# ucas-vg/PointTinyBenchmark

Hardware: AMD Instinct MI355X
Metric: img/s (640x640) CPR R50-FPN fwd+loss (higher is better)
Workload: dtype fp32

## Files before the change

### include/cpr_hip.h

```cpp
#ifndef CPR_HIP_H
#define CPR_HIP_H
#ifdef __cplusplus
extern "C" {
#endif

#define CPR_ERR_ARG (-1001)
#define CPR_ERR_UNSUPPORTED (-1002)

int cpr_version(void);

#define CPR_CONV_RELU 1
#define CPR_CONV_OUT_BF16 2
#define CPR_CONV_RES_MASK 4
#define CPR_CONV_COLSUM 8
int cpr_conv2d_fwd(const float* in, const float* wgt, float* out, const float* scale, const float* bias,
                   const float* residual, const float* in_a, const float* in_b, float* gn_part, int N, int H, int W,
                   int Cin, int Cout, int KH, int KW, int stride, int pad, int Kpad, int flags, int in_relu,
                   int* variant_out, void* stream);
int cpr_conv2d_fwd_dil(const float* in, const float* wgt, float* out, const float* scale, const float* bias,
                       const float* residual, const float* in_a, const float* in_b, float* gn_part, int N, int H, int W,
                       int Cin, int Cout, int KH, int KW, int stride, int pad, int dil, int Kpad, int flags, int in_relu,
                       int* variant_out, void* stream);

int cpr_conv2d_dual_fwd(const float* in, const float* wgt, const float* in2, const float* wgt2, float* out,
                        const float* scale, const float* bias, const float* scale2, const float* bias2, int N, int H, int W,
                        int Cin, int Cout, int KH, int KW, int stride, int pad, int Kpad, int H2, int W2, int Cin2,
                        int stride2, int Kpad2, int flags, int* variant_out, void* stream);

int cpr_conv1x1_stream_fwd(const float* in, const float* wgt, float* out, const float* scale, const float* bias,
                           const float* residual, long long M, int Cin, int Cout, int flags, void* stream);

int cpr_conv_wgrad_bf16_workspace_s(int N, int H, int W, int Cin, int Cout, int k, int stride, int dy_bf16, int x_bf16);
int cpr_conv_wgrad_bf16_s(const void* dy, int dy_bf16, const void* x, int x_bf16, float* grad, void* ws, int N, int H, int W, int Cin,
                          int Cout, int k, int stride, int accumulate, void* stream);

#define CPR_WINO_IN_B8 1
#define CPR_WINO_OUT_B8 2
int cpr_wino_pack_weights(const float* wgt, float* u, int Cin, int Cout, int Kpad, void* stream);
int cpr_conv3x3_wino_fwd(const float* in, const float* u, float* out, const float* scale, const float* bias,
                         const float* in_a, const float* in_b, float* gn_part, int N, int H, int W, int Cin, int Cout,
                         int flags, int in_relu, int layout, void* stream);
int cpr_wino32_pack_weights(const float* wgt, float* u, int Cin, int Cout, int Kpad, void* stream);
int cpr_conv3x3_wino32_slots(int H, int W);
int cpr_conv3x3_wino32_fwd(const float* in, const float* u, float* out, const float* scale, const float* bias,
                           const float* in_a, const float* in_b, float* gn_part, int N, int H, int W, int Cin, int Cout,
                           int flags, int in_relu, int layout, void* stream);
int cpr_gn_apply_b8(const float* x, const float* a, const float* b, float* y, int N, int H, int W, int C, int relu,
                    void* stream);

int cpr_conv2d_fwd_bf16(const void* in, const void* wgt, const void* wgt_frag, void* out, const float* scale, const float* bias,
                        const void* residual, float* gn_part, int N, int H, int W, int Cin, int Cout, int KH, int KW,
                        int stride, int pad, int Kpad, int relu, int out_fp32, int* variant_out, void* stream);
int cpr_conv2d_bf16_mask_slots(int N, int H, int W, int Cin, int Cout, int KH, int KW, int stride, int pad, int out_fp32);
int cpr_conv2d_dgrad_bf16_fused(const void* in, const void* wgt, const void* wgt_frag, float* out32, void* out16, const float* add32,
                                const void* mask, float* part, int N, int H, int W, int Cin, int Cout, int KH, int KW, int stride,
                                int pad, int Kpad, int* variant_out, void* stream);
int cpr_stem7x7s2_bf16(const float* in, const void* wgt, const float* scale, const float* bias, void* out, int N, int H, int W,
                       int relu, int layout, void* stream);
int cpr_stem7x7s2_pool_bf16(const float* in, const void* wgt, const float* scale, const float* bias, void* out, int N, int H,
                            int W, int layout, void* stream);
int cpr_maxpool3x3s2_bf16(const void* in, void* out, int N, int H, int W, int C, void* stream);
int cpr_gn_stats_bf16(const void* x, float* part, int N, int HW, int C, int P, void* stream);
int cpr_gn_apply_bf16(const void* x, const float* a, const float* b, const void* up, void* y, int N, int H, int W,
                      int C, int UH, int UW, int relu, void* stream);

int cpr_nchw_to_nhwc4(const float* in, float* out, int N, int C, int H, int W, void* stream);
int cpr_nhwc_to_nchw(const float* in, float* out, int N, int C, int H, int W, void* stream);
int cpr_stem7x7s2_pool_f32(const float* in, const float* wgt, const float* scale, const float* bias, float* out, int N, int H,
                           int W, int layout, void* stream);
int cpr_maxpool3x3s2(const float* in, float* out, int N, int H, int W, int C, void* stream);
int cpr_stem_deep_fwd(const float* in, const float* w1, const float* s1, const float* b1, const float* w2, const float* s2,
                      const float* b2, const float* w3, const float* s3, const float* b3, float* mid1, float* mid2, void* out, int N,
                      int H, int W, int layout, int out_bf16, void* stream);
int cpr_stem3x3s2_fwd(const float* in, const float* w, const float* scale, const float* bias, float* out, int N, int H, int W,
                      int layout, void* stream);
int cpr_stem3x3s2_wgrad_workspace(int N, int H, int W);
int cpr_stem3x3s2_wgrad(const float* dy, const float* in, float* gw, float* ws, int N, int H, int W, int layout, void* stream);
int cpr_avgpool_fwd(const void* in, void* out, int N, int H, int W, int C, int s, int bf16, void* stream);
int cpr_avgpool_bwd(const void* g, const void* add, void* dx, int N, int H, int W, int C, int s, int bf16, void* stream);
int cpr_maxpool3x3s2_rec(const float* in, float* out, unsigned char* arg, int N, int H, int W, int C, void* stream);
int cpr_maxpool3x3s2_bf16_rec(const void* in, void* out, unsigned char* arg, int N, int H, int W, int C, void* stream);
int cpr_stem7x7s2_pool_f32_rec(const float* in, const float* wgt, const float* scale, const float* bias, float* out,
                               unsigned char* arg, int N, int H, int W, int layout, void* stream);
int cpr_stem7x7s2_pool_bf16_rec(const float* in, const void* wgt, const float* scale, const float* bias, void* out,
                                unsigned char* arg, int N, int H, int W, int layout, void* stream);
int cpr_stem_pool_bwd_blocks(long long M);
int cpr_stem_pool_bwd(const float* dp, const unsigned char* arg, float* dy, float* part, int N, int OH, int OW, void* stream);
int cpr_stem_wgrad_f32_workspace(int N, int H, int W);
int cpr_stem_wgrad_f32(const float* dy, const float* in, float* gw, float* ws, int N, int H, int W, int layout, void* stream);

int cpr_gn_stats(const float* x, float* part, int N, int HW, int C, int P, void* stream);
int cpr_gn_finalize(const float* part, const float* gamma, const float* beta, float* a_out, float* b_out,
                    float* mean_out, float* rstd_out, int N, int P, int C, int G, int HW, float eps, void* stream);
int cpr_gn_apply(const float* x, const float* a, const float* b, const float* up, float* y, int N, int H, int W,
                 int C, int UH, int UW, int relu, void* stream);

int cpr_box_centers(const float* boxes, float* centers, int n, void* stream);

#define CPR_PROB_SIGMOID 0
#define CPR_PROB_SOFTMAX 1
#define CPR_PROB_NORMED_SIGMOID 2
#define CPR_PROB_IDENTITY 3

int cpr_logit_project(const float* x, const float* w, const float* bias, const float* in_a, const float* in_b,
                      float* out, int N, int HW, int Cin, int J, int in_relu, void* stream);

int cpr_neg_mask_loss(const float* logit, int J, const float* centers, const int* labels, const int* gt_start,
                      const int* pad_hw, unsigned char* mask, double* partial, int N, int H, int W, int C,
                      float stride, float d2_thr, float eps, int class_wise, int prob_type, float norm_p,
                      int mask_classes, int* n_partial, void* stream);

int cpr_bag_sample(const float* map, int J, const float* centers, const int* gt_img, const int* pad_hw,
                   const float* offsets, float* pts, unsigned char* valid, float* out, int G, int K, int H, int W,
                   float stride, int align_corners, const float* pad_value, void* stream);

int cpr_grid_bag(const float* map, int J, const float* points, const int* gt_img, int R, int Kmax, float radius_px,
                 const float* pad_value, float* pts, unsigned char* valid, int* ws_cell, int* count, float* out, int G,
                 int H, int W, float stride, int align_corners, void* stream);

int cpr_mil_loss(const float* logits, int J, int ins_off, const unsigned char* valid, const int* labels,
                 const float* gt_weight, float* bag_ws, const double* neg_partial, int n_partial, int num_bags,
                 int bag_stride, int bag_off, int bag_len, int ctr_off, int ctr_stride, int ctr_count, int ctr_mod,
                 int C, float eps, int prob_type, float norm_p, int binary_ins, int allpos, float w_mil, float w_gt,
                 float w_neg, int neg_from_gt, float* out5, void* stream);

int cpr_refine(const float* logits, int J, const float* pts, const unsigned char* valid, const float* centers, int Rv,
               int ctr_stride, const int* labels, const int* gt_img, const int* gt_start, const int* img_hw,
               const unsigned char* not_refine_in, float* refine_pts, float* scores, unsigned char* not_refine,
               unsigned char* chosen, int G, int Kt, int Kv, int C, int prob_type, float norm_p, float gt_alpha,
               float merge_th, float refine_th, int use_nearest, int use_classify, int score_max, void* stream);

int cpr_point_assign(const float* points, const float* gt_bboxes, int n, int k, float scale, int pos_num,
                     long long* gt_inds, float* ws_best, int* ws_lvl, void* stream);

int cpr_hungarian_cost(const float* pred, int pred_stride, const float* logits, int C, const float* gt,
                       const int* labels, float* costT, int M, int G, float w_cls, float alpha, float gamma,
                       float eps, float w_dis, float fx, float fy, int p_norm, void* stream);
int cpr_match_cost(const float* pred, int pdim, const float* logits, int C, const float* gt, const int* labels, float* costT,
                   int M, int G, const float* terms, int ncls, int nreg, void* stream);

int cpr_lsa_topk(const float* costT, const int* m_of, const int* g_of, const long long* cost_off,
                 const long long* col_off, const long long* row_off, int num_problems, int topk, long long* gt_inds,
                 double* ws_v, double* ws_spc, int* ws_path, int* ws_row4col, unsigned char* ws_sc,
                 unsigned char* ws_active, int* ws_cols, int* ws_remaining, int* ws_pos, double* ws_u,
                 int* ws_col4row, unsigned char* ws_sr, int* status, int max_cols, int max_rows, void* stream);

int cpr_topk_desc(const float* scores, int n, int k, float* out_vals, long long* out_idx, void* stream);

int cpr_nms_candidates(const float* boxes, int box_stride, const float* scores, const float* factors, int n, int C,
                       float score_thr, float* cand_boxes, float* cand_scores, int* cand_labels, long long* cand_inds,
                       int* count, void* stream);
int cpr_nms_workspace(int n);
int cpr_nms(const float* boxes, const float* scores, const int* labels, int n, float iou_thr, long long* keep_idx,
            int* num_keep, int* ws_order, float* ws_boxes, unsigned long long* ws_mask, void* stream);
int cpr_topk_desc_batched(const float* scores, int B, int n, int k, float* out_vals, long long* out_idx, void* stream);
int cpr_nms_candidates_batched(const float* boxes, int box_stride, const float* scores, const float* factors, int B, int n,
                               int C, float score_thr, float* cand_boxes, float* cand_scores, int* cand_labels,
                               long long* cand_inds, int* count, void* stream);
int cpr_nms_batched(const float* boxes, const float* scores, const int* labels, const int* n_dev, int B, int cap,
                    float iou_thr, long long* keep_idx, int* num_keep, int* ws_order, float* ws_boxes,
                    unsigned long long* ws_mask, long long ws_stride, void* stream);

int cpr_p2p_decode(const float* reg, const float* point_anchor, float* pred, float* anchor, int N, int H, int W, int k,
                   float stride, float gamma, void* stream);
int cpr_tap_sum3x3(const float* R, const float* bias, float* out, int N, int H, int W, int J, void* stream);
int cpr_rowmax_sigmoid(const float* logits, float* out, long long M, int C, void* stream);
int cpr_sigmoid(const float* x, float* y, long long n, void* stream);
int cpr_p2p_loss(const float* logits, const float* pred, const long long* gt_inds, const float* gt_pts,
                 const int* gt_labels, const int* gt_start, double* ws_partial, float* out, int B, int M, int C,
                 float alpha, float gamma, float beta, float pos_w, float neg_w, float reg_norm, float w_cls,
                 float w_reg, int cls_mode, int reg_mode, void* stream);

int cpr_conv2d_wgrad_workspace(int N, int OH, int OW, int Cin, int Cout, int KH, int KW);
int cpr_conv2d_wgrad(const float* dy, const float* x, const float* in_a, const float* in_b, float* grad_w, float* ws,
                     int N, int H, int W, int Cin, int Cout, int KH, int KW, int stride, int pad, int in_relu,
                     int accumulate, void* stream);
int cpr_conv2d_wgrad_dil(const float* dy, const float* x, float* grad_w, float* ws, int N, int H, int W, int Cin, int Cout, int KH,
                         int KW, int stride, int pad, int dil, int accumulate, void* stream);
int cpr_conv3x3_wino_wgrad_workspace(int N, int H, int W, int Cin, int Cout);
int cpr_conv3x3_wino_wgrad(const float* dy, const float* x, const float* in_a, const float* in_b, float* grad_w, float* ws,
                           int N, int H, int W, int Cin, int Cout, int in_relu, int accumulate, void* stream);
int cpr_gn_bwd(const float* x, const float* dz, const float* a, const float* b, const float* mean, const float* rstd,
               const float* gamma, float* dx, float* dgamma, float* dbeta, float* ws_part, float* ws_k, int N, int HW,
               int C, int G, int P, int relu, int accumulate, void* stream);
int cpr_gn_bwd_bf16(const void* x_bf16, const float* dz, const float* a, const float* b, const float* mean, const float* rstd,
                    const float* gamma, float* dx, void* dx_bf16, float* dgamma, float* dbeta, float* ws_part, float* ws_k, int N,
                    int HW, int C, int G, int P, int relu, int accumulate, void* stream);
int cpr_gn_bwd_bf16_dz16(const void* x_bf16, const void* dz_bf16, const float* a, const float* b, const float* mean, const float* rstd,
                         const float* gamma, float* dx, void* dx_bf16, float* dgamma, float* dbeta, float* ws_part, float* ws_k,
                         int N, int HW, int C, int G, int P, int relu, int accumulate, void* stream);
int cpr_upsample_add_bwd(const float* dfine, float* dcoarse, int N, int H, int W, int UH, int UW, int C, int accumulate,
                         void* stream);
int cpr_relu_bwd_colsum_ws(long long M, int C);
int cpr_relu_bwd_colsum(const float* dy, const float* add, const void* y, int y_bf16, float* g_out, void* g16_out, float* colsum,
                        float* ws_part, long long M, int C, int accumulate, void* stream);
int cpr_part_colsum(const float* part, float* out, float* ws, int tiles, int C, void* stream);
int cpr_bn_fold_bwd(float* Gw, const float* weight, const float* scale, const float* mean, const float* inv_sigma,
                    const float* colsum_g, float* dgamma, float* dbeta, int Cout, int K, void* stream);
int cpr_bn_fold_bwd_part(float* Gw, const float* weight, const float* scale, const float* mean, const float* inv_sigma, const float* part,
                         int tiles, float* dgamma, float* dbeta, int Cout, int K, void* stream);
int cpr_axpby(float* y, const float* x, float alpha, float beta, long long n, void* stream);
int cpr_phase_scatter_add(const float* src, float* dst, int N, int Hs, int Ws, int C, int H, int W, int py, int px,
                          int sh, int sw, int s, void* stream);
int cpr_zero_insert(const float* dy, float* out, int N, int OH, int OW, int C, int H, int W, int s, void* stream);
int cpr_pack_weights_grouped(const float* w, const float* scale, float* out, int C, int cg, int transpose, void* stream);
int cpr_pack_weights_grouped_multi(const void* jobs_dev, int n, int total_blocks, void* stream);
int cpr_conv_group_fwd(const float* x, const float* wp, float* out, const float* scale, const float* bias, int N, int H, int W, int C,
                       int cg, int stride, int flags, void* stream);
int cpr_conv_group_wgrad_workspace(int N, int OH, int OW, int C, int cg);
int cpr_conv_group_wgrad(const float* dy, const float* x, float* grad_w, float* ws, int N, int H, int W, int C, int cg, int stride,
                         int accumulate, void* stream);
int cpr_conv_group_fwd_pitch(const float* x, const float* wp, float* out, const float* scale, const float* bias, int N, int H, int W,
                             int C, int Cp, int cg, int stride, int flags, void* stream);
int cpr_conv_group_wgrad_pitch(const float* dy, const float* x, float* grad_w, float* ws, int N, int H, int W, int C, int Cp, int cg,
                               int stride, int accumulate, void* stream);
int cpr_conv_group_fwd_dil(const float* x, const float* wp, float* out, const float* scale, const float* bias, int N, int H, int W,
                           int C, int cg, int dil, int flags, void* stream);
int cpr_conv_group_wgrad_dil(const float* dy, const float* x, float* grad_w, float* ws, int N, int H, int W, int C, int cg, int dil,
                             int accumulate, void* stream);
int cpr_res2_pack_weights(const float* w, const float* scale, float* out, int width, int transpose, void* stream);
int cpr_res2_conv_fwd(const float* x, int x_pitch, int x_off, const float* add, int add_pitch, int add_off, const float* wp, float* out,
                      int out_pitch, int out_off, const float* scale, const float* bias, int N, int IH, int IW, int OH, int OW, int width,
                      int stride, int transposed, int flags, void* stream);
int cpr_res2_conv_wgrad_workspace(int N, int OH, int OW, int width);
int cpr_res2_conv_wgrad(const float* dy, int dy_pitch, int dy_off, const float* x, int x_pitch, int x_off, const float* add, int add_pitch,
                        int add_off, float* grad_w, float* ws, int N, int H, int W, int width, int stride, int accumulate, void* stream);
int cpr_res2_relu_bwd_colsum(float* g, int g_pitch, int g_off, const float* carry, int c_pitch, int c_off, const float* y, int y_pitch,
                             int y_off, float* colsum, float* ws, long long M, int width, void* stream);
int cpr_res2_pool_fwd(const float* x, int x_pitch, int x_off, float* out, int out_pitch, int out_off, int N, int H, int W, int width,
                      int stride, void* stream);
int cpr_res2_pool_bwd(const float* dy, int dy_pitch, int dy_off, float* dx, int dx_pitch, int dx_off, int N, int H, int W, int width,
                      int stride, void* stream);
int cpr_subsample2(const void* x, int x_bf16, const float* a, const float* b, void* out, int N, int H, int W, int C, void* stream);
int cpr_subsample2_bwd_add(const float* dfine, const float* dcoarse, float* out, int N, int H, int W, int C, void* stream);
int cpr_relu_mask_add(const float* dz, const float* d, const void* y, int y_bf16, float* out, long long n, void* stream);
int cpr_gn_apply2(const float* x1, const float* a1, const float* b1, const float* x2, const float* a2, const float* b2, float* y, int N, int H,
                  int W, int C, void* stream);
int cpr_gn_apply2_bf16(const void* x1, const float* a1, const float* b1, const void* x2, const float* a2, const float* b2, void* y, int N,
                       int H, int W, int C, void* stream);
typedef struct cpr_bfp_level {
    const void* x;
    const float* a;
    const float* b;
    void* y;
    void* arg;
    int H, W;
    float sy, sx;
} cpr_bfp_level;
int cpr_bfp_gather(const cpr_bfp_level* levels, int L, int refine_level, float* bsf, int N, int C, int arg_wide, void* stream);
int cpr_bfp_gather_bf16(const cpr_bfp_level* levels, int L, int refine_level, void* bsf, int N, int C, int arg_wide, void* stream);
int cpr_bfp_scatter(const cpr_bfp_level* levels, int L, int refine_level, const float* ref, const float* ref_a, const float* ref_b, int N,
                    int C, int arg_wide, void* stream);
int cpr_bfp_scatter_bf16(const cpr_bfp_level* levels, int L, int refine_level, const void* ref, const float* ref_a, const float* ref_b,
                         int N, int C, int arg_wide, void* stream);
int cpr_bfp_scatter_bwd(const cpr_bfp_level* levels, int L, int refine_level, float* d_ref, int N, int C, int arg_wide, void* stream);
int cpr_bfp_gather_bwd(const cpr_bfp_level* levels, int L, int refine_level, const float* d_bsf, int N, int C, int arg_wide, void* stream);
int cpr_loss_bwd(const float* lmap, const unsigned char* neg_mask, const float* out5, const float* bag_logits,
                 const unsigned char* valid, const int* labels, const float* gt_weight, const float* bag_ws,
                 const float* centers, const int* gt_img, const float* offsets, float* dbag_ws, float* dmap, float* win_ws,
                 int* win_org, int win, int N, int H, int W, int J, int Jd, int ins_off, int G, int K, int C, float stride,
                 float eps, float w_mil, float w_gt, float w_neg, const float* upstream, void* stream);
int cpr_bag_gather_bwd(const float* dsample, int J, const float* centers, const int* gt_img, const float* offsets,
                       float* win_ws, int* win_org, int win, float* dmap, int N, int H, int W, int Jd, int G, int K,
                       float stride, void* stream);
int cpr_bag_points_gather_bwd(const float* dsample, int J, const float* pts, const int* code, const int* gt_img, float* dmap,
                              float* wout_ws, float* dbias, int N, int H, int W, int Jd, int G, int Kt, float stride,
                              int align_corners, void* stream);
int cpr_loss_bwd_general(const float* lmap, const unsigned char* neg_mask, const float* out5, const float* bag_logits,
                         const unsigned char* valid, const int* labels, const float* gt_weight, const float* bag_ws, float* dbag,
                         float* dmap, int N, int H, int W, int J, int Jd, int ins_off, int num_bags, int bag_stride, int bag_off,
                         int bag_len, int ctr_off, int ctr_stride, int ctr_count, int ctr_mod, int C, float eps, int prob_type,
                         float norm_p, int binary_ins, int allpos, float w_mil, float w_gt, float w_neg, int neg_from_gt,
                         const float* upstream, void* stream);
int cpr_pack_weights(const float* w, const float* scale, float* out, int O, int I, int KH, int KW, int colsp, int Kpad,
                     int transpose, void* stream);
int cpr_pack_weights_bf16(const float* w, const float* scale, void* out, void* frag, int O, int I, int KH, int KW, int transpose,
                          void* stream);
int cpr_spin(long long ticks, void* stream);
int cpr_bn_fold(const float* gamma, const float* beta, const float* mean, const float* var, float eps, float* scale,
                float* shift, float* inv_sigma, int C, void* stream);
int cpr_bn_train_ws(long long M, int C);
int cpr_bn_batch_stats(const float* y, const float* gamma, const float* beta, float* running_mean, float* running_var,
                       long long* num_batches_tracked, float momentum, float eps, float* mean, float* rstd, float* scale, float* shift,
                       float* center, float* cmean, float* cshift, float* ws, long long M, int C, void* stream);
int cpr_bn_apply(const float* y, const float* center, const float* scale, const float* shift, const float* residual, const float* y2,
                 const float* center2, const float* scale2, const float* shift2, float* out, long long M, int C, int relu, void* stream);
int cpr_bn_train_bwd(const float* dout, const float* z, const float* y, const float* center, const float* mean, const float* rstd,
                     const float* gamma, float* dy, float* dgamma, float* dbeta, float* ws, long long M, int C, void* stream);
int cpr_bn_sync_ws(long long M, int C);
int cpr_bn_sync_stats_local(const float* y, double* record, float* ws, long long M, int C, void* stream);
int cpr_bn_sync_stats_merge(const double* records, int R, const float* y, const float* gamma, const float* beta, float* running_mean,
                            float* running_var, long long* num_batches_tracked, float momentum, float eps, float* mean, float* rstd,
                            float* scale, float* shift, float* center, float* cmean, float* cshift, double* count, int C, void* stream);
int cpr_bn_sync_bwd_local(const float* dout, const float* z, const float* y, const float* center, const float* mean, const float* rstd,
                          float* dgamma, float* dbeta, double* record, float* ws, long long M, int C, void* stream);
int cpr_bn_sync_bwd_merge(const double* records, int R, const double* count, const float* dout, const float* z, const float* y,
                          const float* center, const float* mean, const float* rstd, const float* gamma, float* dy, float* ws, long long M,
                          int C, void* stream);
int cpr_p2p_out_bf16_fwd(const void* x, const float* a, const float* b, const float* w, const float* bias, float* taps, float* out,
                         int N, int H, int W, int Cin, int J, void* stream);
int cpr_p2p_out_bf16_dgrad(const float* dout, int ldd, const float* w, void* dx, int out_bf16, int N, int H, int W, int Cin, int J,
                           void* stream);
int cpr_p2p_out_bf16_wgrad_ws(int N, int H, int W, int Cin, int J);
int cpr_p2p_out_bf16_wgrad(const void* x, const float* a, const float* b, const float* dout, int ldd, float* gw, float* gb, float* ws,
                           int N, int H, int W, int Cin, int J, void* stream);
int cpr_bn_fold_multi(const void* jobs_dev, int n, int max_c, void* stream);
int cpr_pack_weights_multi(const void* jobs_dev, int n, int total_blocks, void* stream);
int cpr_pack_weights_bf16_multi(const void* jobs_dev, int n, int total_blocks, void* stream);
int cpr_p2p_loss_bwd(const float* logits, const float* pred, const long long* gt_inds, const float* gt_pts,
                     const int* gt_labels, const int* gt_start, const float* npos, float* dcls, float* dreg, int B, int M,
                     int C, int Cp, int Rp, float alpha, float gamma, float beta, float pos_w, float neg_w, float reg_norm,
                     float w_cls, float w_reg, float gamma_p, const float* upstream, int cls_mode, int reg_mode, void* stream);
int cpr_p2p_loss_bwd_levels(const float* logits, const float* pred, const long long* gt_inds, const float* gt_pts,
                            const int* gt_labels, const int* gt_start, const float* npos, int B, int M, int C, int P, int L,
                            const int* level_hw, const int* level_off, const int* level_cp, const int* level_rp,
                            float* const* level_dcls, float* const* level_dreg, float alpha, float gamma, float beta, float pos_w,
                            float neg_w, float reg_norm, float w_cls, float w_reg, float gamma_p, const float* upstream,
                            int cls_mode, int reg_mode, void* stream);
int cpr_grad_sumsq(const float* g, long long n, double* ws_partial, double* out, int accumulate, void* stream);
int cpr_sgd_step(float* p, const float* grad, float* buf, const double* norm2, long long n, float lr, float mu, float wd,
                 float max_norm, float grad_scale, int first, void* stream);
int cpr_adam_step(float* p, const float* grad, float* exp_avg, float* exp_avg_sq, const double* norm2, long long n, double lr,
                  double beta1, double beta2, double eps, double wd, float step_size, float bc2_sqrt, float max_norm,
                  float grad_scale, int decoupled, void* stream);

int cpr_preprocess_u8(const unsigned char* img, const int* flip, const float* mean3, const float* stdinv3, int to_rgb,
                      float* out, int N, int H, int W, int Hp, int Wp, void* stream);
int cpr_clip_flip_boxes(float* boxes, const int* img_of, const int* flip, const int* img_hw, int n, int clip,
                        void* stream);

typedef struct cpr_preprocess_job {
    const unsigned char* src;
    long long out_off;
    double scale_x, scale_y;
    int pitch, src_w, src_h, x0, y0, cw, ch, dw, dh, flip, Hp, Wp;
} cpr_preprocess_job;
int cpr_preprocess_jobs_u8(const void* jobs_dev, int n_jobs, const float* mean3, const float* stdinv3, int to_rgb, float* out,
                           long long total_out_pixels, void* stream);
int cpr_scale_clip_flip_boxes(float* boxes, const int* img_of, const int* flip, const int* img_hw, const float* scale4, int n,
                              int clip, void* stream);

#ifdef CPR_BENCH_HOOKS
int cpr_conv_force_tile(int bm, int bn);
int cpr_conv_set_pipeline(int mode);
// ... 18 lines not shown
```

### pointtinybenchmark_amd/_lib.py

```python
import ctypes
import os

_HERE = os.path.dirname(os.path.abspath(__file__))
LIB_PATH = os.path.join(_HERE, 'csrc', 'libcprhip.so')

_p = ctypes.c_void_p
_i = ctypes.c_int
_f = ctypes.c_float
_l = ctypes.c_longlong
_d = ctypes.c_double

SIGNATURES = {
    'cpr_version': [],
    'cpr_conv2d_fwd': [_p, _p, _p, _p, _p, _p, _p, _p, _p, _i, _i, _i, _i, _i, _i, _i, _i, _i, _i, _i, _i, _p, _p],
    'cpr_conv2d_fwd_dil': [_p] * 9 + [_i] * 13 + [_p, _p],
    'cpr_conv2d_dual_fwd': [_p] * 9 + [_i] * 16 + [_p, _p],
    'cpr_conv1x1_stream_fwd': [_p, _p, _p, _p, _p, _p, _l, _i, _i, _i, _p],
    'cpr_conv_wgrad_bf16_workspace_s': [_i] * 9,
    'cpr_conv_wgrad_bf16_s': [_p, _i, _p, _i, _p, _p] + [_i] * 8 + [_p],
    'cpr_wino_pack_weights': [_p, _p, _i, _i, _i, _p],
    'cpr_conv3x3_wino_fwd': [_p, _p, _p, _p, _p, _p, _p, _p, _i, _i, _i, _i, _i, _i, _i, _i, _p],
    'cpr_wino32_pack_weights': [_p, _p, _i, _i, _i, _p],
    'cpr_conv3x3_wino32_slots': [_i, _i],
    'cpr_conv3x3_wino32_fwd': [_p, _p, _p, _p, _p, _p, _p, _p, _i, _i, _i, _i, _i, _i, _i, _i, _p],
    'cpr_conv3x3_wino_wgrad_workspace': [_i, _i, _i, _i, _i],
    'cpr_conv3x3_wino_wgrad': [_p, _p, _p, _p, _p, _p, _i, _i, _i, _i, _i, _i, _i, _p],
    'cpr_gn_apply_b8': [_p, _p, _p, _p, _i, _i, _i, _i, _i, _p],
    'cpr_conv2d_fwd_bf16': [_p, _p, _p, _p, _p, _p, _p, _p] + [_i] * 12 + [_p, _p],
    'cpr_conv2d_bf16_mask_slots': [_i] * 10,
    'cpr_bn_fold_multi': [_p, _i, _i, _p],
    'cpr_pack_weights_multi': [_p, _i, _i, _p],
    'cpr_pack_weights_bf16_multi': [_p, _i, _i, _p],
    'cpr_conv2d_dgrad_bf16_fused': [_p] * 8 + [_i] * 10 + [_p, _p],
    'cpr_stem7x7s2_bf16': [_p, _p, _p, _p, _p, _i, _i, _i, _i, _i, _p],
    'cpr_stem7x7s2_pool_bf16': [_p, _p, _p, _p, _p, _i, _i, _i, _i, _p],
    'cpr_maxpool3x3s2_bf16': [_p, _p, _i, _i, _i, _i, _p],
    'cpr_gn_stats_bf16': [_p, _p, _i, _i, _i, _i, _p],
    'cpr_gn_apply_bf16': [_p, _p, _p, _p, _p, _i, _i, _i, _i, _i, _i, _i, _p],
    'cpr_nchw_to_nhwc4': [_p, _p, _i, _i, _i, _i, _p],
    'cpr_nhwc_to_nchw': [_p, _p, _i, _i, _i, _i, _p],
    'cpr_stem7x7s2_pool_f32': [_p, _p, _p, _p, _p, _i, _i, _i, _i, _p],
    'cpr_maxpool3x3s2': [_p, _p, _i, _i, _i, _i, _p],
    'cpr_stem_deep_fwd': [_p] * 13 + [_i] * 5 + [_p],
    'cpr_stem3x3s2_fwd': [_p] * 5 + [_i] * 4 + [_p],
    'cpr_stem3x3s2_wgrad_workspace': [_i, _i, _i],
    'cpr_stem3x3s2_wgrad': [_p, _p, _p, _p, _i, _i, _i, _i, _p],
    'cpr_avgpool_fwd': [_p, _p] + [_i] * 6 + [_p],
    'cpr_avgpool_bwd': [_p, _p, _p] + [_i] * 6 + [_p],
    'cpr_maxpool3x3s2_rec': [_p, _p, _p, _i, _i, _i, _i, _p],
    'cpr_maxpool3x3s2_bf16_rec': [_p, _p, _p, _i, _i, _i, _i, _p],
    'cpr_stem7x7s2_pool_f32_rec': [_p, _p, _p, _p, _p, _p, _i, _i, _i, _i, _p],
    'cpr_stem7x7s2_pool_bf16_rec': [_p, _p, _p, _p, _p, _p, _i, _i, _i, _i, _p],
    'cpr_stem_pool_bwd_blocks': [_l],
    'cpr_stem_pool_bwd': [_p, _p, _p, _p, _i, _i, _i, _p],
    'cpr_stem_wgrad_f32_workspace': [_i, _i, _i],
    'cpr_stem_wgrad_f32': [_p, _p, _p, _p, _i, _i, _i, _i, _p],
    'cpr_gn_stats': [_p, _p, _i, _i, _i, _i, _p],
    'cpr_gn_finalize': [_p, _p, _p, _p, _p, _p, _p, _i, _i, _i, _i, _i, _f, _p],
    'cpr_gn_apply': [_p, _p, _p, _p, _p, _i, _i, _i, _i, _i, _i, _i, _p],
    'cpr_box_centers': [_p, _p, _i, _p],
    'cpr_logit_project': [_p, _p, _p, _p, _p, _p, _i, _i, _i, _i, _i, _p],
    'cpr_neg_mask_loss': [_p, _i, _p, _p, _p, _p, _p, _p, _i, _i, _i, _i, _f, _f, _f, _i, _i, _f, _i, _p, _p],
    'cpr_bag_sample': [_p, _i, _p, _p, _p, _p, _p, _p, _p, _i, _i, _i, _i, _f, _i, _p, _p],
    'cpr_grid_bag': [_p, _i, _p, _p, _i, _i, _f, _p, _p, _p, _p, _p, _p, _i, _i, _i, _f, _i, _p],
    'cpr_mil_loss': [_p, _i, _i, _p, _p, _p, _p, _p] + [_i] * 10 + [_f, _i, _f, _i, _i, _f, _f, _f, _i, _p, _p],
    'cpr_refine': [_p, _i, _p, _p, _p, _i, _i] + [_p] * 9 + [_i, _i, _i, _i, _i, _f, _f, _f, _f, _i, _i, _i, _p],
    'cpr_point_assign': [_p, _p, _i, _i, _f, _i, _p, _p, _p, _p],
    'cpr_hungarian_cost': [_p, _i, _p, _i, _p, _p, _p, _i, _i, _f, _f, _f, _f, _f, _f, _f, _i, _p],
    'cpr_lsa_topk': [_p, _p, _p, _p, _p, _p, _i, _i] + [_p] * 14 + [_i, _i, _p],
    'cpr_topk_desc': [_p, _i, _i, _p, _p, _p],
    'cpr_nms_candidates': [_p, _i, _p, _p, _i, _i, _f, _p, _p, _p, _p, _p, _p],
    'cpr_nms_workspace': [_i],
    'cpr_nms': [_p, _p, _p, _i, _f, _p, _p, _p, _p, _p, _p],
    'cpr_topk_desc_batched': [_p, _i, _i, _i, _p, _p, _p],
    'cpr_nms_candidates_batched': [_p, _i, _p, _p, _i, _i, _i, _f, _p, _p, _p, _p, _p, _p],
    'cpr_tap_sum3x3': [_p, _p, _p, _i, _i, _i, _i, _p],
    'cpr_nms_batched': [_p, _p, _p, _p, _i, _i, _f, _p, _p, _p, _p, _p, _l, _p],
    'cpr_p2p_decode': [_p, _p, _p, _p, _i, _i, _i, _i, _f, _f, _p],
    'cpr_rowmax_sigmoid': [_p, _p, ctypes.c_longlong, _i, _p],
    'cpr_sigmoid': [_p, _p, ctypes.c_longlong, _p],
    'cpr_p2p_loss': [_p, _p, _p, _p, _p, _p, _p, _p, _i, _i, _i, _f, _f, _f, _f, _f, _f, _f, _f, _i, _i, _p],
    'cpr_match_cost': [_p, _i, _p, _i, _p, _p, _p, _i, _i, _p, _i, _i, _p],
    'cpr_conv2d_wgrad_workspace': [_i] * 7,
    'cpr_conv2d_wgrad': [_p] * 6 + [_i] * 11 + [_p],
    'cpr_conv2d_wgrad_dil': [_p] * 4 + [_i] * 11 + [_p],
    'cpr_gn_bwd': [_p] * 12 + [_i] * 7 + [_p],
    'cpr_gn_bwd_bf16': [_p] * 13 + [_i] * 7 + [_p],
    'cpr_gn_bwd_bf16_dz16': [_p] * 13 + [_i] * 7 + [_p],
    'cpr_upsample_add_bwd': [_p, _p] + [_i] * 7 + [_p],
    'cpr_relu_bwd_colsum_ws': [_l, _i],
    'cpr_relu_bwd_colsum': [_p, _p, _p, _i, _p, _p, _p, _p, _l, _i, _i, _p],
    'cpr_bn_fold_bwd': [_p] * 8 + [_i, _i, _p],
    'cpr_bn_fold_bwd_part': [_p, _p, _p, _p, _p, _p, _i, _p, _p, _i, _i, _p],
    'cpr_part_colsum': [_p, _p, _p, _i, _i, _p],
    'cpr_axpby': [_p, _p, _f, _f, _l, _p],
    'cpr_phase_scatter_add': [_p, _p] + [_i] * 11 + [_p],
    'cpr_zero_insert': [_p, _p] + [_i] * 7 + [_p],
    'cpr_subsample2': [_p, _i, _p, _p, _p, _i, _i, _i, _i, _p],
    'cpr_subsample2_bwd_add': [_p, _p, _p, _i, _i, _i, _i, _p],
    'cpr_relu_mask_add': [_p, _p, _p, _i, _p, _l, _p],
    'cpr_gn_apply2': [_p] * 7 + [_i] * 4 + [_p],
    'cpr_gn_apply2_bf16': [_p] * 7 + [_i] * 4 + [_p],
    'cpr_bfp_gather': [_p, _i, _i, _p, _i, _i, _i, _p],
    'cpr_bfp_gather_bf16': [_p, _i, _i, _p, _i, _i, _i, _p],
    'cpr_bfp_scatter': [_p, _i, _i, _p, _p, _p, _i, _i, _i, _p],
    'cpr_bfp_scatter_bf16': [_p, _i, _i, _p, _p, _p, _i, _i, _i, _p],
    'cpr_bfp_scatter_bwd': [_p, _i, _i, _p, _i, _i, _i, _p],
    'cpr_bfp_gather_bwd': [_p, _i, _i, _p, _i, _i, _i, _p],
    'cpr_loss_bwd': [_p] * 15 + [_i] * 10 + [_f] * 5 + [_p, _p],
    'cpr_bag_gather_bwd': [_p, _i, _p, _p, _p, _p, _p, _i, _p, _i, _i, _i, _i, _i, _i, _f, _p],
    'cpr_bag_points_gather_bwd': [_p, _i, _p, _p, _p, _p, _p, _p, _i, _i, _i, _i, _i, _i, _f, _i, _p],
    'cpr_loss_bwd_general': [_p] * 10 + [_i] * 15 + [_f, _i, _f, _i, _i, _f, _f, _f, _i, _p, _p],
    'cpr_preprocess_u8': [_p, _p, _p, _p, _i, _p, _i, _i, _i, _i, _i, _p],
    'cpr_clip_flip_boxes': [_p, _p, _p, _p, _i, _i, _p],
    'cpr_preprocess_jobs_u8': [_p, _i, _p, _p, _i, _p, _l, _p],
    'cpr_scale_clip_flip_boxes': [_p, _p, _p, _p, _p, _i, _i, _p],
    'cpr_pack_weights': [_p, _p, _p] + [_i] * 7 + [_p],
    'cpr_pack_weights_bf16': [_p, _p, _p, _p] + [_i] * 5 + [_p],
    'cpr_pack_weights_grouped': [_p, _p, _p, _i, _i, _i, _p],
    'cpr_pack_weights_grouped_multi': [_p, _i, _i, _p],
    'cpr_conv_group_fwd': [_p] * 5 + [_i] * 7 + [_p],
    'cpr_conv_group_wgrad_workspace': [_i] * 5,
    'cpr_conv_group_wgrad': [_p] * 4 + [_i] * 7 + [_p],
    'cpr_conv_group_fwd_pitch': [_p] * 5 + [_i] * 8 + [_p],
    'cpr_conv_group_wgrad_pitch': [_p] * 4 + [_i] * 8 + [_p],
    'cpr_conv_group_fwd_dil': [_p] * 5 + [_i] * 7 + [_p],
    'cpr_conv_group_wgrad_dil': [_p] * 4 + [_i] * 7 + [_p],
    'cpr_res2_pack_weights': [_p, _p, _p, _i, _i, _p],
    'cpr_res2_conv_fwd': [_p, _i, _i, _p, _i, _i, _p, _p, _i, _i, _p, _p] + [_i] * 9 + [_p],
    'cpr_res2_conv_wgrad_workspace': [_i] * 4,
    'cpr_res2_conv_wgrad': [_p, _i, _i, _p, _i, _i, _p, _i, _i, _p, _p] + [_i] * 6 + [_p],
    'cpr_res2_pool_fwd': [_p, _i, _i, _p, _i, _i] + [_i] * 5 + [_p],
    'cpr_res2_relu_bwd_colsum': [_p, _i, _i, _p, _i, _i, _p, _i, _i, _p, _p, _l, _i, _p],
    'cpr_res2_pool_bwd': [_p, _i, _i, _p, _i, _i] + [_i] * 5 + [_p],
    'cpr_spin': [ctypes.c_longlong, _p],
    'cpr_bn_fold': [_p, _p, _p, _p, _f, _p, _p, _p, _i, _p],
    'cpr_bn_train_ws': [_l, _i],
    'cpr_bn_batch_stats': [_p] * 6 + [_f, _f] + [_p] * 8 + [_l, _i, _p],
    'cpr_bn_apply': [_p] * 10 + [_l, _i, _i, _p],
    'cpr_bn_train_bwd': [_p] * 11 + [_l, _i, _p],
    'cpr_bn_sync_ws': [_l, _i],
    'cpr_bn_sync_stats_local': [_p, _p, _p, _l, _i, _p],
    'cpr_bn_sync_stats_merge': [_p, _i] + [_p] * 6 + [_f, _f] + [_p] * 8 + [_i, _p],
    'cpr_bn_sync_bwd_local': [_p] * 10 + [_l, _i, _p],
    'cpr_bn_sync_bwd_merge': [_p, _i] + [_p] * 10 + [_l, _i, _p],
    'cpr_p2p_out_bf16_fwd': [_p] * 7 + [_i] * 5 + [_p],
    'cpr_p2p_out_bf16_dgrad': [_p, _i, _p, _p] + [_i] * 6 + [_p],
    'cpr_p2p_out_bf16_wgrad_ws': [_i] * 5,
    'cpr_p2p_out_bf16_wgrad': [_p] * 4 + [_i] + [_p] * 3 + [_i] * 5 + [_p],
    'cpr_p2p_loss_bwd': [_p] * 9 + [_i] * 5 + [_f] * 9 + [_p, _i, _i, _p],
    'cpr_p2p_loss_bwd_levels': [_p] * 7 + [_i] * 5 + [_p] * 6 + [_f] * 9 + [_p, _i, _i, _p],
    'cpr_grad_sumsq': [_p, _l, _p, _p, _i, _p],
    'cpr_sgd_step': [_p, _p, _p, _p, _l, _f, _f, _f, _f, _f, _i, _p],
    'cpr_adam_step': [_p, _p, _p, _p, _p, _l, _d, _d, _d, _d, _d, _f, _f, _f, _f, _i, _p],
}

BENCH_SIGNATURES = {
    'cpr_lsa_phase_clocks': [_p, _i],
    'cpr_wino32_set_debug': [_i, _i, _i],
    'cpr_conv_force_tile': [_i, _i],
    'cpr_conv_set_pipeline': [_i],
    'cpr_conv_set_stream': [_i],
    'cpr_conv_set_ablation': [_i],
    'cpr_wgrad_set_ablation': [_i],
    'cpr_wino_set_variant': [_i, _i],
    'cpr_wino_set_staging': [_i, _i],
    'cpr_conv_set_extra_lds': [_i],
    'cpr_bf16_set_dma': [_i],
    'cpr_bf16_set_wfrag': [_i],
    'cpr_bn_set_finalize_only': [_i],
}
BENCH_LIB_PATH = os.path.join(_HERE, 'csrc', 'libcprhip_bench.so')

_lib = None


class CprHipError(RuntimeError):
    pass


def load():
    global _lib
    if _lib is not None:
        return _lib
    path, sigs = LIB_PATH, dict(SIGNATURES)
    if os.environ.get('CPR_BENCH_HOOKS', '0') == '1':
        path = BENCH_LIB_PATH
        sigs.update(BENCH_SIGNATURES)
    if not os.path.exists(path):
        raise CprHipError('%s not found: run `python -m pointtinybenchmark_amd.build%s` (no CPU fallback exists)'
                          % (path, ' --bench-hooks' if path == BENCH_LIB_PATH else ''))
    lib = ctypes.CDLL(path)
    for name, argtypes in sigs.items():
        fn = getattr(lib, name, None)
        if fn is None:
            raise CprHipError('symbol %s missing from %s (stale build?)' % (name, path))
        fn.argtypes = argtypes
        fn.restype = ctypes.c_int
    _lib = lib
    return lib


def call(name, *args, positive=False):
    rc = getattr(load(), name)(*args)
    if positive and rc >= 0:
        return rc
    if rc != 0:
        if rc == -1001:
            raise CprHipError('%s: invalid argument' % name)
        if rc == -1002:
            raise CprHipError('%s: unsupported configuration' % name)
        raise CprHipError('%s failed with hipError %d' % (name, -rc))
    return rc
```

### pointtinybenchmark_amd/csrc/conv_wino.hip

```cpp
#include <type_traits>
#include "common.h"

typedef float f32x2 __attribute__((ext_vector_type(2)));
typedef int i32x4 __attribute__((ext_vector_type(4)));
typedef float f32x2 __attribute__((ext_vector_type(2)));

__device__ __forceinline__ f32x2 pk_add(f32x2 a, f32x2 b) {
    f32x2 r; asm("v_pk_add_f32 %0, %1, %2" : "=v"(r) : "v"(a), "v"(b)); return r;
}
__device__ __forceinline__ f32x2 pk_sub(f32x2 a, f32x2 b) {
    f32x2 r; asm("v_pk_add_f32 %0, %1, %2 neg_lo:[0,1] neg_hi:[0,1]" : "=v"(r) : "v"(a), "v"(b)); return r;
}
__device__ __forceinline__ f32x2 pk_col01(f32x2 t01, f32x2 t23) {
    f32x2 r; asm("v_pk_add_f32 %0, %1, %2 op_sel:[0,0] op_sel_hi:[1,0] neg_lo:[0,1] neg_hi:[0,0]" : "=v"(r) : "v"(t01), "v"(t23)); return r;
}
__device__ __forceinline__ f32x2 pk_col23(f32x2 t01, f32x2 t23) {
    f32x2 r; asm("v_pk_add_f32 %0, %1, %2 op_sel:[1,0] op_sel_hi:[1,1] neg_lo:[1,0] neg_hi:[0,1]" : "=v"(r) : "v"(t01), "v"(t23)); return r;
}
__device__ __forceinline__ f32x2 pk_fma(f32x2 a, f32x2 b, f32x2 c) {
    f32x2 r; asm("v_pk_fma_f32 %0, %1, %2, %3" : "=v"(r) : "v"(a), "v"(b), "v"(c)); return r;
}

struct WinoParams {
    const float* in;
    const float* u;
    float* out;
    const float* scale;
    const float* bias;
    float* gn_part;
    const float* in_a;
    const float* in_b;
    int in_relu, out_b8;
    int N, H, W, Cin, Cout, relu, RY, RX, regions, tilesN, nch;
    int tpx;
};

constexpr int WBUF = 16 * 64 * 8;

__global__ void wino_pack_kernel(const float* __restrict__ w, float* __restrict__ u, int Cin, int Cout, int Kpad) {
    const int idx = blockIdx.x * blockDim.x + threadIdx.x;
    if (idx >= Cin * Cout) return;
    const int ci = idx % Cin, co = idx / Cin;
    float g[3][3];
#pragma unroll
    for (int a = 0; a < 3; ++a)
#pragma unroll
        for (int b = 0; b < 3; ++b) g[a][b] = w[(size_t)co * Kpad + (a * 3 + b) * Cin + ci];
    float t[4][3];
#pragma unroll
    for (int b = 0; b < 3; ++b) {
        t[0][b] = g[0][b];
        t[1][b] = 0.5f * (g[0][b] + g[1][b] + g[2][b]);
        t[2][b] = 0.5f * (g[0][b] - g[1][b] + g[2][b]);
        t[3][b] = g[2][b];
    }
    const int tn = co >> 6, cl = co & 63, chunk = ci >> 3, k = ci & 7, nch = Cin >> 3;
    float* dst = u + ((size_t)(tn * nch + chunk) * 16) * 512 + cl * 8 + 4 * ((k >> 2) ^ ((cl >> 3) & 1)) + (k & 3);
#pragma unroll
    for (int i = 0; i < 4; ++i) {
        dst[(i * 4 + 0) * 512] = t[i][0];
        dst[(i * 4 + 1) * 512] = 0.5f * (t[i][0] + t[i][1] + t[i][2]);
        dst[(i * 4 + 2) * 512] = 0.5f * (t[i][0] - t[i][1] + t[i][2]);
        dst[(i * 4 + 3) * 512] = t[i][2];
    }
}

template <int ABL, bool INB8, bool XF, int TSPREAD = 1, int VAR = 0>
__global__ __launch_bounds__(512, 1) void conv_wino_kernel(WinoParams p) {
    constexpr bool DEEP = (VAR & 1) != 0, UDMA = (VAR & 4) != 0, USINGLE = (VAR & 2) != 0 && !UDMA;
    constexpr int XFMAX = 512;
    constexpr int RAWROW = 148;
    constexpr int RAWBUF = 18 * RAWROW;
    __shared__ __attribute__((aligned(16))) float smem[4 * WBUF + 2 * RAWBUF + (XF ? 4 * XFMAX : 0)];
    float* Vs = smem;
    float* Us = smem + 2 * WBUF;

    const int tid = threadIdx.x, lane = tid & 63;
    const int wave = __builtin_amdgcn_readfirstlane(tid >> 6);
    const int wi = wave & 3;
    const int nh = wave >> 2;

    const int pixbytes = INB8 ? 32 : p.Cin * 4;
    const int chunk_bytes = INB8 ? p.H * p.W * 32 : 32;
    const __amdgpu_buffer_rsrc_t rs_in = __builtin_amdgcn_make_buffer_rsrc(
        const_cast<float*>(p.in), 0, (int)((size_t)p.N * p.H * p.W * p.Cin * 4), 0x00020000);
    const __amdgpu_buffer_rsrc_t rs_u = __builtin_amdgcn_make_buffer_rsrc(
        const_cast<float*>(p.u), 0, (int)((size_t)p.tilesN * p.nch * WBUF * 4), 0x00020000);
    float* Rw = smem + 4 * WBUF;
    float* ABs = smem + 4 * WBUF + 2 * RAWBUF;
    int par = 0;
    int upyx[2], raw_wr[2];
#pragma unroll
    for (int k = 0; k < 2; ++k) {
        const int pix = (tid + 512 * k) >> 1;
        const int py = pix / 18, px = pix - py * 18;
        upyx[k] = py << 8 | px;
        raw_wr[k] = py * RAWROW + px * 8 + (tid & 1) * 4;
    }
    const bool second_unit = wave < 3;
    const bool unit1_live = tid + 512 < 648;
    const int lch = tid & 7, tyl = (tid >> 3) & 7, ltile = wave * 8 + tyl;
    const float* t_rd = Rw + (2 * tyl) * RAWROW + (2 * wave) * 8 + lch;
    const int v_wr = ltile * 8 + 4 * ((lch >> 2) ^ ((ltile >> 3) & 1)) + (lch & 3);
    const int last = p.nch - 1;
    const float relu_floor = (XF && p.in_relu) ? 0.f : -INFINITY;

    struct Tile {
        int rg, tn, n, oy0, ox0, n0;
        int voffA[2];
        unsigned uok;
        bool any_pad, valid;
    };
    const int T = p.regions * p.tilesN;
    const int per = (T + 7) >> 3;
    const int ngrp = p.tpx > 0 ? p.tilesN / p.tpx : 1;
    const int per_r = p.tpx > 0 ? (p.regions * ngrp + 7) / 8 : 0;
    auto setup = [&](int vb) {
        Tile t;
        if (p.tpx > 0) {
            const int x = vb & 7, s = vb >> 3;
            const int sr = s / p.tpx;
            t.rg = (x / ngrp) * per_r + sr;
            t.tn = (x % ngrp) * p.tpx + (s - sr * p.tpx);
            t.valid = sr < per_r && t.rg < p.regions;
            if (!t.valid) { t.rg = 0; t.tn = 0; }
        } else {
            const int tile = (vb & 7) * per + (vb >> 3);
            t.valid = vb < per * 8 && tile < T;
            const int tl = t.valid ? tile : 0;
            t.rg = tl / p.tilesN; t.tn = tl - t.rg * p.tilesN;
        }
        t.n = t.rg / (p.RY * p.RX);
        const int rrem = t.rg - t.n * p.RY * p.RX;
        const int ry = rrem / p.RX, rx = rrem - ry * p.RX;
        t.oy0 = ry * 16; t.ox0 = rx * 16; t.n0 = t.tn * 64;
        const int img_base = INB8 ? (t.n * (p.Cin >> 3)) * p.H * p.W * 32 : t.n * p.H * p.W * p.Cin * 4;
        t.uok = 0;
#pragma unroll
        for (int k = 0; k < 2; ++k) {
            const int iy = t.oy0 - 1 + (upyx[k] >> 8), ix = t.ox0 - 1 + (upyx[k] & 255);
            const bool ok = (k == 0 || unit1_live) & ((unsigned)iy < (unsigned)p.H) & ((unsigned)ix < (unsigned)p.W);
            t.uok |= (ok ? 1u : 0u) << k;
            t.voffA[k] = ok ? img_base + (iy * p.W + ix) * pixbytes + (tid & 1) * 16 : (int)0x80000000;
        }
        t.any_pad = XF && __builtin_amdgcn_ballot_w64(t.uok != (unit1_live ? 3u : 1u)) != 0;
        return t;
    };

    f32x4 sp[2][2];
    f32x4 su[(USINGLE || UDMA) ? 1 : 2][4];
    float tab_a = 0.f, tab_b = 0.f;
    f32x2 d[4][2];
    if (ABL & 9) { sp[0][0] = f32x4{1.f, 1.f, 1.f, 1.f}; sp[0][1] = sp[0][0]; sp[1][0] = sp[0][0]; sp[1][1] = sp[0][0]; }
    Tile cur = setup(blockIdx.x);
    auto ld_a = [&](const Tile& t, int ck, int k) {
        return __builtin_bit_cast(f32x4, __builtin_amdgcn_raw_buffer_load_b128(rs_in, t.voffA[k], ck * chunk_bytes, 0));
    };
    auto ld_u = [&](const Tile& t, int ck, int z) {
        return __builtin_bit_cast(
            f32x4, __builtin_amdgcn_raw_buffer_load_b128(rs_u, tid * 16 + z * 8192, (t.tn * p.nch + ck) * (WBUF * 4), 0));
    };
    auto prefetch = [&](const Tile& t) {
        if (!(ABL & 8)) {
            sp[0][0] = ld_a(t, 0, 0); sp[1][0] = ld_a(t, 1, 0);
            if (second_unit) { sp[0][1] = ld_a(t, 0, 1); sp[1][1] = ld_a(t, 1, 1); }
        }
        if (!UDMA) {
#pragma unroll
            for (int z = 0; z < 4; ++z) { su[0][z] = ld_u(t, 0, z); if (!USINGLE) su[USINGLE ? 0 : 1][z] = ld_u(t, 1, z); }
        }
        if (XF) {
            if (tid < p.Cin) { tab_a = p.in_a[t.n * p.Cin + tid]; tab_b = p.in_b[t.n * p.Cin + tid]; }
        }
    };
    auto g_a = [&](auto set_c, int chunk, int k) {
        constexpr int SET = decltype(set_c)::value;
        if (ABL & 8) return;
        const int ck = chunk < last ? chunk : last;
        if (k == 0 || second_unit) sp[SET][k] = ld_a(cur, ck, k);
    };
    auto g_u = [&](auto set_c, int chunk, int z) {
        constexpr int SET = (USINGLE || UDMA) ? 0 : decltype(set_c)::value;
        if (!UDMA) su[SET][z] = ld_u(cur, chunk < last ? chunk : last, z);
    };
    const int lds_u0 = (int)(unsigned)(size_t)(smem + 2 * WBUF);
    const size_t u_addr = (size_t)p.u;
    const i32x4 rs_u_raw = {(int)(unsigned)u_addr, (int)(unsigned)(u_addr >> 32) & 0xffff,
                            (int)((size_t)p.tilesN * p.nch * WBUF * 4), 0x00020000};
    auto dma_u = [&](int chunk, int buf, int z) {
        const int soff = (cur.tn * p.nch + chunk) * (WBUF * 4);
        const int m0v = lds_u0 + buf * (WBUF * 4) + z * 8192 + wave * 1024;
        asm volatile("s_nop 4\n\ts_mov_b32 m0, %0\n\ts_nop 0\n\tbuffer_load_dwordx4 %1, %2, %3 offen offset:0 lds"
                     :: "s"(m0v), "v"(tid * 16 + z * 8192), "s"(rs_u_raw), "s"(soff) : "memory");
    };
    auto dma_wait = [&](auto npatch_c) {
        constexpr int NP = decltype(npatch_c)::value;
        if (NP == 0) asm volatile("s_waitcnt vmcnt(0)" ::: "memory");
        else if (second_unit) asm volatile("s_waitcnt vmcnt(%0)" :: "n"(2 * NP) : "memory");
        else asm volatile("s_waitcnt vmcnt(%0)" :: "n"(NP) : "memory");
    };
    auto affine = [&](f32x4 v, f32x4 a4, f32x4 b4, int k) {
        if (ABL & 64) v = v * a4 + b4;
        else {
            const f32x2 lo = pk_fma(f32x2{v.x, v.y}, f32x2{a4.x, a4.y}, f32x2{b4.x, b4.y});
            const f32x2 hi = pk_fma(f32x2{v.z, v.w}, f32x2{a4.z, a4.w}, f32x2{b4.z, b4.w});
            v = f32x4{lo.x, lo.y, hi.x, hi.y};
        }
        v.x = fmaxf(v.x, relu_floor); v.y = fmaxf(v.y, relu_floor); v.z = fmaxf(v.z, relu_floor); v.w = fmaxf(v.w, relu_floor);
        if (cur.any_pad) {
            asm volatile("");
            if (!((cur.uok >> k) & 1u)) v = f32x4{0.f, 0.f, 0.f, 0.f};
        }
        return v;
    };
    f32x4 xa4, xb4;
    auto xf_fetch = [&](int chunk) {
        const float* tab = ABs + par * 2 * XFMAX + (chunk < last ? chunk : last) * 8 + (tid & 1) * 4;
        xa4 = *reinterpret_cast<const f32x4*>(tab);
        xb4 = *reinterpret_cast<const f32x4*>(tab + XFMAX);
    };
    auto r_a = [&](auto set_c, int buf, int k) {
        constexpr int SET = decltype(set_c)::value;
        if (k == 1 && !second_unit) return;
        f32x4 v = sp[SET][k];
        if (XF) v = affine(v, xa4, xb4, k);
        if (k == 0 || unit1_live) *reinterpret_cast<f32x4*>(Rw + buf * RAWBUF + raw_wr[k]) = v;
    };
    auto r_a_pro = [&](int chunk01, int k) {
        if (k == 1 && !second_unit) return;
        f32x4 v = chunk01 ? sp[1][k] : sp[0][k];
        if (XF) {
            const float* tab = ABs + par * 2 * XFMAX + chunk01 * 8 + (tid & 1) * 4;
            v = affine(v, *reinterpret_cast<const f32x4*>(tab), *reinterpret_cast<const f32x4*>(tab + XFMAX), k);
        }
        if (k == 0 || unit1_live) *reinterpret_cast<f32x4*>(Rw + chunk01 * RAWBUF + raw_wr[k]) = v;
    };
    auto r_u = [&](auto set_c, int buf, int z) {
        constexpr int SET = (USINGLE || UDMA) ? 0 : decltype(set_c)::value;
        if (!UDMA) *reinterpret_cast<f32x4*>(Us + buf * WBUF + tid * 4 + z * 2048) = su[SET][z];
    };
    auto t_read = [&](int buf, int r) {
#pragma unroll
        for (int s = 0; s < 2; ++s)
            d[r][s] = f32x2{t_rd[buf * RAWBUF + r * RAWROW + (2 * s) * 8], t_rd[buf * RAWBUF + r * RAWROW + (2 * s + 1) * 8]};
    };
    auto t_row = [&](int buf, int i) {
        float* dst = Vs + buf * WBUF + (i * 4) * 512 + v_wr;
        if (ABL & 64) {
            float ts[4];
#pragma unroll
            for (int s = 0; s < 4; ++s) {
                const float d0 = d[0][s >> 1][s & 1], d1 = d[1][s >> 1][s & 1], d2 = d[2][s >> 1][s & 1], d3 = d[3][s >> 1][s & 1];
                ts[s] = i == 0 ? d0 - d2 : i == 1 ? d1 + d2 : i == 2 ? d2 - d1 : d1 - d3;
            }
            dst[0 * 512] = ts[0] - ts[2];
            dst[1 * 512] = ts[1] + ts[2];
            dst[2 * 512] = ts[2] - ts[1];
            dst[3 * 512] = ts[1] - ts[3];
            return;
        }
        f32x2 t[2];
#pragma unroll
        for (int s = 0; s < 2; ++s)
            t[s] = i == 0 ? pk_sub(d[0][s], d[2][s]) : i == 1 ? pk_add(d[1][s], d[2][s]) : i == 2 ? pk_sub(d[2][s], d[1][s])
                                                                                                  : pk_sub(d[1][s], d[3][s]);
        const f32x2 o01 = pk_col01(t[0], t[1]), o23 = pk_col23(t[0], t[1]);
        dst[0 * 512] = o01.x;
        dst[1 * 512] = o01.y;
        dst[2 * 512] = o23.x;
        dst[3 * 512] = o23.y;
    };
    const int l31 = lane & 31, half = lane >> 5;
    const float* a_lds = Vs + (wi * 4 * 64 + l31) * 8 + 4 * (half ^ ((l31 >> 3) & 1));
    const float* b_lds = Us + (wi * 4 * 64 + nh * 32 + l31) * 8 + 4 * (half ^ ((l31 >> 3) & 1));
    using Set0 = std::integral_constant<int, 0>;
    using Set1 = std::integral_constant<int, 1>;

    if (cur.valid) prefetch(cur);
    if (XF) {
        if (tid < p.Cin) { ABs[tid] = tab_a; ABs[XFMAX + tid] = tab_b; }
        __syncthreads();
    }
    for (int vb = blockIdx.x; cur.valid; vb += gridDim.x) {
    const int rg = cur.rg, n = cur.n, oy0 = cur.oy0, ox0 = cur.ox0, n0 = cur.n0;

    f32x16 acc[4][2];
#pragma unroll
    for (int j = 0; j < 4; ++j)
#pragma unroll
        for (int tb = 0; tb < 2; ++tb)
#pragma unroll
            for (int r = 0; r < 16; ++r) acc[j][tb][r] = 0.f;

    f32x4 fa0[2], fb0, fa1[2], fb1;
#define WFRAG(FA, FB, buf, j, z)                                                                                    \
    do {                                                                                                            \
        if ((z) < 2) FA[(z) < 2 ? (z) : 0] = *reinterpret_cast<const f32x4*>(a_lds + (buf) * WBUF + (j) * 512 + ((z) < 2 ? (z) : 0) * 256); \
        else FB = *reinterpret_cast<const f32x4*>(b_lds + (buf) * WBUF + (j) * 512);                                \
    } while (0)
#define WMFMA(FA, FB, j, q) \
    acc[j][(q) & 1] = __builtin_amdgcn_mfma_f32_32x32x2f32(FA[(q) & 1][(q) >> 1], FB[(q) >> 1], acc[j][(q) & 1], 0, 0, 0)
    r_a_pro(0, 0); r_a_pro(0, 1);
    r_a_pro(1, 0); r_a_pro(1, 1);
    if (UDMA) {
#pragma unroll
        for (int z = 0; z < 4; ++z) dma_u(0, 0, z);
#pragma unroll
        for (int z = 0; z < 4; ++z) dma_u(1, 1, z);
    }
#pragma unroll
    for (int z = 0; z < 4; ++z) r_u(Set0{}, 0, z);
    g_a(Set0{}, 2, 0); g_a(Set0{}, 2, 1);
    if (DEEP) { g_a(Set1{}, 3, 0); g_a(Set1{}, 3, 1); }
#pragma unroll
    for (int z = 0; z < 4; ++z) g_u(Set0{}, USINGLE ? 1 : 2, z);
    __syncthreads();
#pragma unroll
    for (int r = 0; r < 4; ++r) t_read(0, r);
#pragma unroll
    for (int i = 0; i < 4; ++i) t_row(0, i);
    if (TSPREAD == 1) {
#pragma unroll
        for (int r = 0; r < 4; ++r) t_read(1, r);
    }
    if (UDMA) dma_wait(std::integral_constant<int, DEEP ? 2 : 1>{});
    __syncthreads();
#pragma unroll
    for (int z = 0; z < 3; ++z) WFRAG(fa0, fb0, 0, 0, z);

    auto iteration = [&](auto nxt_c, int c) {
        const int buf = c & 1;
        const std::integral_constant<int, DEEP ? 1 - decltype(nxt_c)::value : 0> pset_c{};
#pragma unroll
        for (int q = 0; q < 8; ++q) {
            WMFMA(fa0, fb0, 0, q);
            if (q < 3 && !(ABL & 2)) WFRAG(fa1, fb1, buf, 1, q);
            if (!(ABL & 1)) {
                if (TSPREAD == 0 || TSPREAD == 2) { if (q >= 4) t_read(buf ^ 1, q - 4); }
                else { if (q == 3) t_row(buf ^ 1, 0); if (q == 6) t_row(buf ^ 1, 1); }
            }
            __builtin_amdgcn_sched_barrier(0);
        }
#pragma unroll
        for (int q = 0; q < 8; ++q) {
            WMFMA(fa1, fb1, 1, q);
            if (q < 3 && !(ABL & 2)) WFRAG(fa0, fb0, buf, 2, q);
            if (!(ABL & 1)) {
                if (q & 1) r_u(nxt_c, buf ^ 1, q >> 1);
                else if (TSPREAD == 0) t_row(buf ^ 1, q >> 1);
                else if (TSPREAD == 2) {
                    if (q == 0) {
#pragma unroll
                        for (int i = 0; i < 4; ++i) t_row(buf ^ 1, i);
                    }
                }
                else if (q == 2) t_row(buf ^ 1, 2);
                else if (q == 6) t_row(buf ^ 1, 3);
                if (XF && q == 7) xf_fetch(c + 2);
            }
            __builtin_amdgcn_sched_barrier(0);
        }
#pragma unroll
        for (int q = 0; q < 8; ++q) {
            WMFMA(fa0, fb0, 2, q);
            if (q < 3 && !(ABL & 2)) WFRAG(fa1, fb1, buf, 3, q);
            if (!(ABL & 1)) {
                if (q == 3) { r_a(pset_c, buf, 0); if (TSPREAD == 2) r_a(pset_c, buf, 1); }
                if (q == 4 && TSPREAD != 2) r_a(pset_c, buf, 1);
                if (q == 5 || q == 6 || q == 7) g_u(nxt_c, c + (USINGLE ? 2 : 3), q - 5);
            }
            __builtin_amdgcn_sched_barrier(0);
        }
        asm volatile("" ::: "memory");
        if (UDMA) dma_wait(std::integral_constant<int, DEEP ? 1 : 0>{});
        __builtin_amdgcn_s_waitcnt(0xc07f);
        if (!(ABL & 4)) __builtin_amdgcn_s_barrier();
        asm volatile("" ::: "memory");
        __builtin_amdgcn_sched_barrier(0);
#pragma unroll
        for (int q = 0; q < 8; ++q) {
            WMFMA(fa1, fb1, 3, q);
            if (q < 3 && !(ABL & 2)) WFRAG(fa0, fb0, buf ^ 1, 0, q);
            if (!(ABL & 1)) {
                if (UDMA) {
                    if (q < 4 && c + 2 < p.nch) dma_u(c + 2, buf, q);
                    if (q == 4) g_a(pset_c, c + (DEEP ? 4 : 3), 0);
                    if (q == 6) g_a(pset_c, c + (DEEP ? 4 : 3), 1);
                } else {
                    if (q == 3) g_a(pset_c, c + (DEEP ? 4 : 3), 0);
                    if (q == 5) g_a(pset_c, c + (DEEP ? 4 : 3), 1);
                    if (q == 7) g_u(nxt_c, c + (USINGLE ? 2 : 3), 3);
                }
                if (TSPREAD == 1 && q >= 4) t_read(buf, q - 4);
            }
            __builtin_amdgcn_sched_barrier(0);
        }
    };
    for (int c = 0; c < p.nch; c += 2) {
        iteration(Set1{}, c);
        iteration(Set0{}, c + 1);
    }
#undef WFRAG
#undef WMFMA

    if (ABL & 32) {
        asm volatile("" ::"v"(acc[0][0]), "v"(acc[0][1]), "v"(acc[1][0]), "v"(acc[1][1]));
        asm volatile("" ::"v"(acc[2][0]), "v"(acc[2][1]), "v"(acc[3][0]), "v"(acc[3][1]));
        cur = setup(vb + gridDim.x);
        if (cur.valid) prefetch(cur);
        if (XF && tid < p.Cin) { ABs[(par ^ 1) * 2 * XFMAX + tid] = tab_a; ABs[(par ^ 1) * 2 * XFMAX + XFMAX + tid] = tab_b; }
        par ^= 1;
        __syncthreads();
        continue;
    }
    const Tile nxt = setup(vb + gridDim.x);
    if (nxt.valid) prefetch(nxt);
    __syncthreads();
    float* Rs = smem;
#pragma unroll
    for (int tb = 0; tb < 2; ++tb)
#pragma unroll
        for (int r = 0; r < 16; ++r) {
            const int trow = tb * 32 + (r & 3) + 8 * (r >> 2) + 4 * half;
            const float m0 = acc[0][tb][r], m1 = acc[1][tb][r], m2 = acc[2][tb][r], m3 = acc[3][tb][r];
            Rs[((wi * 2 + 0) * 64 + trow) * 64 + nh * 32 + l31] = m0 + m1 + m2;
            Rs[((wi * 2 + 1) * 64 + trow) * 64 + nh * 32 + l31] = m1 - m2 - m3;
        }
    __syncthreads();
    const int c4 = tid & 15;
    const int co = n0 + c4 * 4;
    f32x4 sc = {1.f, 1.f, 1.f, 1.f}, bi = {0.f, 0.f, 0.f, 0.f};
    if (p.scale) sc = *reinterpret_cast<const f32x4*>(p.scale + co);
    if (p.bias) bi = *reinterpret_cast<const f32x4*>(p.bias + co);
    const __amdgpu_buffer_rsrc_t rs_out = __builtin_amdgcn_make_buffer_rsrc(
        p.out, 0, (int)((size_t)p.N * p.H * p.W * p.Cout * 4), 0x00020000);
    f32x4 gs = {0.f, 0.f, 0.f, 0.f}, gq = {0.f, 0.f, 0.f, 0.f};
#pragma unroll
    for (int k = 0; k < 2; ++k) {
        const int t = (tid >> 4) + 32 * k;
        const int oy = oy0 + 2 * (t & 7), ox = ox0 + 2 * (t >> 3);
#pragma unroll
        for (int b = 0; b < 2; ++b) {
            const f32x4 r0 = *reinterpret_cast<const f32x4*>(Rs + ((0 * 2 + b) * 64 + t) * 64 + c4 * 4);
            const f32x4 r1 = *reinterpret_cast<const f32x4*>(Rs + ((1 * 2 + b) * 64 + t) * 64 + c4 * 4);
            const f32x4 r2 = *reinterpret_cast<const f32x4*>(Rs + ((2 * 2 + b) * 64 + t) * 64 + c4 * 4);
            const f32x4 r3 = *reinterpret_cast<const f32x4*>(Rs + ((3 * 2 + b) * 64 + t) * 64 + c4 * 4);
            f32x4 y[2] = {r0 + r1 + r2, r1 - r2 - r3};
#pragma unroll
            for (int a = 0; a < 2; ++a) {
                f32x4 v = y[a] * sc + bi;
                if (p.relu) { v.x = fmaxf(v.x, 0.f); v.y = fmaxf(v.y, 0.f); v.z = fmaxf(v.z, 0.f); v.w = fmaxf(v.w, 0.f); }
                const bool ok = (oy + a < p.H) & (ox + b < p.W);
                const unsigned off = !ok ? 0x80000000u
                    : p.out_b8 ? (unsigned)((((n * (p.Cout >> 3) + (co >> 3)) * p.H + oy + a) * p.W + ox + b) * 8 + (co & 7)) * 4u
                               : (unsigned)(((n * p.H + oy + a) * p.W + ox + b) * p.Cout + co) * 4u;
                if (!(ABL & 16)) __builtin_amdgcn_raw_buffer_store_b128(__builtin_bit_cast(__attribute__((ext_vector_type(4))) unsigned, v), rs_out, (int)off, 0, 0);
                if (p.gn_part && ok) { gs += v; gq += v * v; }
            }
        }
    }
    if (p.gn_part) {
#pragma unroll
        for (int e = 0; e < 4; ++e) {
            gs[e] += __shfl_xor(gs[e], 16, 64); gs[e] += __shfl_xor(gs[e], 32, 64);
            gq[e] += __shfl_xor(gq[e], 16, 64); gq[e] += __shfl_xor(gq[e], 32, 64);
        }
        __syncthreads();
        if (lane < 16) {
#pragma unroll
            for (int e = 0; e < 4; ++e) {
                smem[(wave * 64 + c4 * 4 + e) * 2 + 0] = gs[e];
                smem[(wave * 64 + c4 * 4 + e) * 2 + 1] = gq[e];
            }
        }
        __syncthreads();
        if (tid < 64) {
            float s = 0.f, q = 0.f;
#pragma unroll
            for (int w8 = 0; w8 < 8; ++w8) { s += smem[(w8 * 64 + tid) * 2]; q += smem[(w8 * 64 + tid) * 2 + 1]; }
            float* dst = p.gn_part + ((size_t)rg * p.Cout + n0 + tid) * 2;
            dst[0] = s; dst[1] = q;
        }
    }
    if (XF && tid < p.Cin) {
        ABs[(par ^ 1) * 2 * XFMAX + tid] = tab_a;
        ABs[(par ^ 1) * 2 * XFMAX + XFMAX + tid] = tab_b;
    }
    par ^= 1;
    __syncthreads();
    cur = nxt;
    }
}

#ifdef CPR_BENCH_HOOKS
static int wino_sched = 0, wino_ablate = 0, wino_var = -1, wino_tpx = -1;
extern "C" int cpr_wino_set_variant(int sched, int ablate) {
    CPR_CHECK_ARG(sched >= 0 && sched <= 2 && ablate >= 0 && ablate <= 64);
    wino_sched = sched;
    wino_ablate = ablate;
    return CPR_OK;
}
extern "C" int cpr_wino_set_staging(int var, int tpx) {
    CPR_CHECK_ARG(var >= -1 && var <= 5 && tpx >= -1 && tpx <= 2);
    wino_var = var;
    wino_tpx = tpx;
    return CPR_OK;
}
#else
constexpr int wino_sched = 0, wino_ablate = 0, wino_var = -1, wino_tpx = -1;
#endif
constexpr int WINO_VAR_DEFAULT = 4, WINO_TPX_DEFAULT = 0;
extern "C" int cpr_wino_pack_weights(const float* wgt, float* u, int Cin, int Cout, int Kpad, hipStream_t stream) {
    CPR_CHECK_ARG(wgt && u && Cin > 0 && Cout > 0 && Cin % 8 == 0 && Cout % 64 == 0 && Kpad >= 9 * Cin);
    hipLaunchKernelGGL(wino_pack_kernel, dim3(cdiv(Cin * Cout, 256)), dim3(256), 0, stream, wgt, u, Cin, Cout, Kpad);
    CPR_LAUNCH_STATUS();
}
static int wino_fwd_launch(const float* in, const float* u, float* out, const float* scale, const float* bias,
                           const float* in_a, const float* in_b, float* gn_part, int N, int H, int W, int Cin,
                           int Cout, int flags, int in_relu, int layout, hipStream_t stream) {
    CPR_CHECK_ARG(in && u && out && N > 0 && H > 0 && W > 0);
    CPR_CHECK_ARG(Cin > 0 && Cout > 0 && Cin % 16 == 0 && Cout % 64 == 0 && Cin >= 32);
    CPR_CHECK_ARG((flags & ~CPR_CONV_RELU) == 0 && (layout & ~3) == 0);
    if (in_a) CPR_CHECK_ARG(in_b && Cin <= 512);
    if ((long long)N * H * W * Cin * 4 >= (1ll << 31) || (long long)N * H * W * Cout * 4 >= (1ll << 31)) return CPR_ERR_UNSUPPORTED;
    WinoParams p;
    p.in = in; p.u = u; p.out = out; p.scale = scale; p.bias = bias; p.gn_part = gn_part;
    p.in_a = in_a; p.in_b = in_b; p.in_relu = in_relu; p.out_b8 = (layout & CPR_WINO_OUT_B8) ? 1 : 0;
    p.N = N; p.H = H; p.W = W; p.Cin = Cin; p.Cout = Cout; p.relu = flags & CPR_CONV_RELU;
    p.RY = (H + 15) / 16; p.RX = (W + 15) / 16;
    p.regions = N * p.RY * p.RX; p.tilesN = Cout / 64; p.nch = Cin / 8;
    const long long T = (long long)p.regions * p.tilesN;
    if (T >= (1ll << 30)) return CPR_ERR_UNSUPPORTED;
    static int cu_of_device[64] = {};
    int dev = 0, ncu = 256;
    if (hipGetDevice(&dev) == hipSuccess && dev >= 0 && dev < 64) {
        if (cu_of_device[dev] == 0) {
            int v = 0;
            if (hipDeviceGetAttribute(&v, hipDeviceAttributeMultiprocessorCount, dev) == hipSuccess && v > 0) cu_of_device[dev] = v;
        }
        if (cu_of_device[dev] > 0) ncu = cu_of_device[dev];
    }
    ncu = (ncu + 7) / 8 * 8;
    int grid = (int)((T + 7) / 8 * 8);
    if (grid > ncu) grid = ncu;
    const bool b8 = (layout & CPR_WINO_IN_B8) != 0, xf = in_a != nullptr;
    p.tpx = wino_tpx >= 0 ? wino_tpx : WINO_TPX_DEFAULT;
    if (p.tpx > 0 && !(p.tilesN % p.tpx == 0 && 8 % (p.tilesN / p.tpx) == 0)) p.tpx = 0;
    if (p.tpx > 0) {
        const long long per_r = ((long long)p.regions * (p.tilesN / p.tpx) + 7) / 8;
        const long long vbs = 8 * per_r * p.tpx;
        if (vbs < grid) grid = (int)vbs;
    }
    const int var = wino_var >= 0 ? wino_var : WINO_VAR_DEFAULT;
#define WLAUNCHV(A_, F_, V_)                                                                                                      \
    do {                                                                                                                         \
        constexpr int TX_ = F_ == 2 ? 2 : 0 ^ F_, TP_ = F_ == 2 ? 2 : 1 ^ F_;                                                     \
        if (b8 && xf) hipLaunchKernelGGL((conv_wino_kernel<A_, true, true, TX_, V_>), dim3(grid), dim3(512), 0, stream, p);       \
        else if (b8) hipLaunchKernelGGL((conv_wino_kernel<A_, true, false, TP_, V_>), dim3(grid), dim3(512), 0, stream, p);       \
        else if (xf) hipLaunchKernelGGL((conv_wino_kernel<A_, false, true, TX_, V_>), dim3(grid), dim3(512), 0, stream, p);       \
        else hipLaunchKernelGGL((conv_wino_kernel<A_, false, false, TP_, V_>), dim3(grid), dim3(512), 0, stream, p);              \
    } while (0)
#define WLAUNCH(A_, F_) WLAUNCHV(A_, F_, WINO_VAR_DEFAULT)
#ifdef CPR_BENCH_HOOKS
    if ((var != WINO_VAR_DEFAULT || wino_sched == 2) && !wino_ablate) {
        switch (var * 3 + wino_sched) {
            case 0: WLAUNCHV(0, 0, 0); break;
            case 1: WLAUNCHV(0, 1, 0); break;
            case 2: WLAUNCHV(0, 2, 0); break;
            case 6: WLAUNCHV(0, 0, 2); break;
            case 7: WLAUNCHV(0, 1, 2); break;
            case 8: WLAUNCHV(0, 2, 2); break;
            case 9: WLAUNCHV(0, 0, 3); break;
            case 10: WLAUNCHV(0, 1, 3); break;
            case 11: WLAUNCHV(0, 2, 3); break;
            case 12: WLAUNCHV(0, 0, 4); break;
            case 13: WLAUNCHV(0, 1, 4); break;
            case 14: WLAUNCHV(0, 2, 4); break;
            default: return CPR_ERR_UNSUPPORTED;
        }
    } else if (wino_ablate || wino_sched) {
        switch (wino_ablate) {
            case 0: WLAUNCH(0, 1); break;
            case 1: WLAUNCH(1, 0); break;
            case 2: WLAUNCH(2, 0); break;
            case 4: WLAUNCH(4, 0); break;
            case 8: WLAUNCH(8, 0); break;
            case 16: WLAUNCH(16, 0); break;
            case 32: WLAUNCH(32, 0); break;
            case 64: WLAUNCH(64, 0); break;
            default: WLAUNCH(7, 0); break;
        }
    } else
#endif
    WLAUNCH(0, 0);
#undef WLAUNCH
#undef WLAUNCHV
    CPR_LAUNCH_STATUS();
}

extern "C" int cpr_conv3x3_wino_fwd(const float* in, const float* u, float* out, const float* scale, const float* bias,
                                    const float* in_a, const float* in_b, float* gn_part, int N, int H, int W, int Cin,
                                    int Cout, int flags, int in_relu, int layout, hipStream_t stream) {
    CPR_CHECK_ARG(N > 0 && H > 0 && W > 0 && Cin > 0 && Cout > 0);
    const int per = cpr_images_per_launch(N, (long long)H * W * cpr_max2(Cin, Cout) * 4);
    if (per <= 0) return CPR_ERR_UNSUPPORTED;
    const size_t slots = (size_t)((H + 15) / 16) * ((W + 15) / 16);
    for (int n0 = 0; n0 < N; n0 += per) {
        const int n = N - n0 < per ? N - n0 : per;
        const int rc = wino_fwd_launch(in + (size_t)n0 * H * W * Cin, u, out + (size_t)n0 * H * W * Cout, scale, bias,
                                       in_a ? in_a + (size_t)n0 * Cin : nullptr, in_b ? in_b + (size_t)n0 * Cin : nullptr,
                                       gn_part ? gn_part + (size_t)n0 * slots * Cout * 2 : nullptr, n, H, W, Cin, Cout, flags,
                                       in_relu, layout, stream);
        if (rc != CPR_OK) return rc;
    }
    return CPR_OK;
}
```

### pointtinybenchmark_amd/layers.py

```python
import struct

import torch
import torch.nn as nn

from . import _lib, ops


_WEIGHT_EPOCH = [0]


def bump_weight_epoch():
    _WEIGHT_EPOCH[0] += 1


REFRESH_IN_PLACE = [True]

_FOLDS, _PACKS16, _PACKS32 = 'cpr_bn_fold_multi', 'cpr_pack_weights_bf16_multi', 'cpr_pack_weights_multi'
_PACKSG = 'cpr_pack_weights_grouped_multi'


class FoldJob:
    multi = _FOLDS
    fold = None
    _ROW = struct.Struct('<7Qif')

    def __init__(self, bn, value):
        self.bn, self.value, self.C = bn, value, bn.weight.numel()
        self._tensors = (bn.weight, bn.bias, bn.running_mean, bn.running_var) + tuple(value)

    def ptrs(self):
        return tuple(map(torch.Tensor.data_ptr, self._tensors))

    def row(self, ptrs, extent):
        return self._ROW.pack(*ptrs, 0, self.C, self.bn.eps), max(extent, self.C)


class PackJob:
    _ROW16, _ROW32 = struct.Struct('<4Q8i'), struct.Struct('<3Q10i')

    def __init__(self, weight, value, transpose, fold):
        self.weight, self.value, self.transpose, self.fold = weight, value, transpose, fold
        self.shape = O, I, KH, KW = weight.shape
        rows, cols = (I, O) if transpose else (O, I)
        bf16 = value.dtype == torch.bfloat16
        self.multi = _PACKS16 if bf16 else _PACKS32
        self.nblocks = max(1, min(64, (rows * (KH * KW * cols // 2 if bf16 else value.Kpad) + 255) // 256))

    def ptrs(self):
        pc = self.value
        return (self.weight.data_ptr(), 0 if self.fold is None else self.fold.value[0].data_ptr(), pc.w.data_ptr(),
                0 if pc.wfrag is None else pc.wfrag.data_ptr())

    def row(self, ptrs, block0):
        pc, nb = self.value, self.nblocks
        if self.multi is _PACKS16:
            return self._ROW16.pack(*ptrs, *self.shape, self.transpose, block0, nb, 0), block0 + nb
        return self._ROW32.pack(*ptrs[:3], nb, 0, *self.shape, pc.Cin, pc.Kpad, self.transpose, block0), block0 + nb

    def refresh_images(self, stream):
        pc = self.value
        for img, fn in ((pc.wino, 'cpr_wino_pack_weights'), (pc.wino32, 'cpr_wino32_pack_weights')):
            if img is not None:
                _lib.call(fn, pc.w.data_ptr(), img.data_ptr(), pc.Cin, pc.Cout, pc.Kpad, stream)


class GroupPackJob(PackJob):
    multi = _PACKSG
    _ROWG = struct.Struct('<3Q6i')

    def __init__(self, weight, value, transpose, fold):
        self.weight, self.value, self.transpose, self.fold = weight, value, transpose, fold
        self.shape = tuple(weight.shape)
        self.nblocks = max(1, min(64, (value.w.numel() + 255) // 256))

    def ptrs(self):
        return (self.weight.data_ptr(), 0 if self.fold is None else self.fold.value[0].data_ptr(), self.value.w.data_ptr())

    def row(self, ptrs, block0):
        pc, nb = self.value, self.nblocks
        return self._ROWG.pack(*ptrs, pc.C, pc.cg, self.transpose, block0, nb, 0), block0 + nb


def _pack_job(pc, weight, transpose=0, fold=None):
    if isinstance(pc, ops.PackedConv) and weight.is_cuda and weight.dtype == torch.float32 and weight.is_contiguous():
        return (GroupPackJob if pc.groups > 1 else PackJob)(weight, pc, transpose, fold)
    return None


class _Entry:
    __slots__ = ('tensors', 'ver', 'val', 'ready')

    def __init__(self, tensors, ver, val, ready):
        self.tensors, self.ver, self.val, self.ready = tensors, ver, val, ready


class _PackCache:

    def __init__(self):
        self._d = {}
        self._jobs = {}
        self._tables = None

    @staticmethod
    def _ver(tensors):
        ver = tuple((t.data_ptr(), t._version) for t in tensors)
        if any(t.requires_grad for t in tensors):
            ver = ver + (_WEIGHT_EPOCH[0],)
        return ver

    def get(self, key, tensors, make, refresh=None):
        ver = self._ver(tensors)
        hit = self._d.get(key)
        if hit is not None and hit.ver == ver:
            hit.ready = ops.wait_ready(hit.ready)
            return hit.val
        val = make()
        job = refresh(val) if refresh is not None else None
        if self._jobs.pop(key, None) is not None or job is not None:
            self._tables = None
        if job is not None:
            self._jobs[key] = job
        self._d[key] = _Entry(list(tensors), ver, val, ops.record_ready())
        return val

    def _live(self):
        if not REFRESH_IN_PLACE[0]:
            return []
        live = [(self._d[k], j) for k, j in self._jobs.items() if self._d[k].val is j.value]
        jobs = {j for _, j in live}
        return [(e, j) for e, j in live if j.fold is None or j.fold in jobs]

    def refresh_all(self):
        live = self._live()
        if not live:
            return
        ptrs = [j.ptrs() for _, j in live]
        if self._tables is None or self._tables[0] != ptrs:
            rows = {_FOLDS: [], _PACKS16: [], _PACKS32: [], _PACKSG: []}
            extent = dict.fromkeys(rows, 0)
            for (_, j), p in zip(live, ptrs):
                row, extent[j.multi] = j.row(p, extent[j.multi])
                rows[j.multi].append(row)
            dev = live[0][0].tensors[0].device
            self._tables = ptrs, [(fn, torch.frombuffer(bytearray(b''.join(r)), dtype=torch.uint8).to(dev), len(r), extent[fn])
                                  for fn, r in rows.items() if r]
        stream = torch.cuda.current_stream().cuda_stream
        for fn, table, n, ext in self._tables[1]:
            _lib.call(fn, table.data_ptr(), n, ext, stream)
        for _, j in live:
            if j.multi is _PACKS32:
                j.refresh_images(stream)
        ready = ops.record_ready()
        for e, j in live:
            e.ver, e.ready = self._ver(e.tensors), ready
            if isinstance(j, PackJob):
                j.value.ready = ready


def packed_conv(cache, conv, dtype=torch.float32):
    return cache.get(('pc', id(conv), dtype), [conv.weight],
                     lambda: ops.PackedConv(conv.weight, conv.stride[0], conv.padding[0], dtype, groups=conv.groups,
                                            dilation=conv.dilation[0]),
                     lambda pc: _pack_job(pc, conv.weight))


def packed_conv_padded_in(cache, conv, Ip):
    O, I = conv.weight.shape[:2]
    assert Ip == ops.pad32(I) and Ip != I, (Ip, I)

    def pack():
        w = torch.zeros((O, Ip) + tuple(conv.weight.shape[2:]), device=conv.weight.device, dtype=torch.float32)
        w[:, :I].copy_(conv.weight.detach())
        return ops.PackedConv(w, conv.stride[0], conv.padding[0])
    return cache.get(('pc_padin', id(conv), Ip), [conv.weight], pack)


def folded_bn(cache, bn):
    def make():
        if bn.weight.is_cuda:
            return ops.bn_fold(bn.weight, bn.bias, bn.running_mean, bn.running_var, bn.eps)[:2]
        with torch.no_grad():
            scale = (bn.weight / torch.sqrt(bn.running_var + bn.eps)).float().contiguous()
            shift = (bn.bias - bn.running_mean * scale).float().contiguous()
        return scale, shift
    def job(val):
        ok = bn.weight.is_cuda and all(t.dtype == torch.float32 and t.is_contiguous()
                                       for t in (bn.weight, bn.bias, bn.running_mean, bn.running_var, val[0], val[1]))
        return FoldJob(bn, val) if ok else None
    return cache.get(('bn', id(bn)), [bn.weight, bn.bias, bn.running_mean, bn.running_var], make, job)


def bn_inv_sigma(cache, bn):
    return cache.get(('bn_is', id(bn)), [bn.running_var],
                     lambda: ops.bn_fold(bn.weight, bn.bias, bn.running_mean, bn.running_var, bn.eps, True)[2])


def dgrad_packed(cache, conv, bn=None, dtype=torch.float32, pitch=None):
    w, stride, pad, dil = conv.weight, conv.stride[0], conv.padding[0], conv.dilation[0]
    if pitch is not None and pitch != w.shape[0]:
        assert bn is not None and conv.groups > 1 and dtype == torch.float32

        def make_p():
            scale, _ = folded_bn(cache, bn)
            return ops.dgrad_pack(w, stride, pad, scale=scale, groups=conv.groups, pitch=pitch)

        def job_p(pc):
            fold = cache._jobs.get(('bn', id(bn)))
            return None if fold is None else _pack_job(pc, w, 1, fold)
        return cache.get(('dgrad', id(conv), dtype, pitch), [w, bn.weight, bn.running_var], make_p, job_p)
    if bn is None:
        return cache.get(('dgrad_raw', id(conv)), [w], lambda: ops.dgrad_pack(w, stride, pad, groups=conv.groups, dilation=dil),
                         lambda pc: _pack_job(pc, w, 1))

    def make():
        scale, _ = folded_bn(cache, bn)
        if dtype == torch.float32 or stride != 1 or conv.groups > 1 or dil != 1:
            return ops.dgrad_pack(w, stride, pad, scale=scale, dtype=dtype, groups=conv.groups, dilation=dil)
        return ops.PackedConv.for_dgrad_bf16(w, pad, scale=scale)

    def job(pc):
        fold = cache._jobs.get(('bn', id(bn)))
        return None if fold is None else _pack_job(pc, w, 1, fold)
    return cache.get(('dgrad', id(conv), dtype), [w, bn.weight, bn.running_var], make, job)


class ConvModule(nn.Module):

    def __init__(self, in_channels, out_channels, kernel_size, stride=1, padding=0, bias='auto', conv_cfg=None,
                 norm_cfg=None, act_cfg=dict(type='ReLU'), inplace=True):
        super().__init__()
        assert conv_cfg is None or conv_cfg.get('type') in (None, 'Conv2d'), 'only plain Conv2d is on this path'
        self.with_norm = norm_cfg is not None
        self.with_activation = act_cfg is not None
        if bias == 'auto':
            bias = not self.with_norm
        self.conv = nn.Conv2d(in_channels, out_channels, kernel_size, stride, padding, bias=bias)
        self.norm_name = None
        if self.with_norm:
            cfg = dict(norm_cfg)
            t = cfg.pop('type')
            rg = cfg.pop('requires_grad', True)
            if t == 'GN':
                self.norm_name = 'gn'
                norm = nn.GroupNorm(num_channels=out_channels, **cfg)
            elif t == 'BN':
                self.norm_name = 'bn'
                norm = nn.BatchNorm2d(out_channels, **cfg)
            else:
                raise KeyError(t)
            for p in norm.parameters():
                p.requires_grad = rg
            self.add_module(self.norm_name, norm)
        if self.with_activation:
            assert act_cfg.get('type', 'ReLU') == 'ReLU'

    @property
    def norm(self):
        return getattr(self, self.norm_name) if self.norm_name else None


def conv_gn(cache, m, x, in_ab=None, in_relu=False, materialize=True, up=None, save=None, consume_input=False,
            out_b8=False):
    gn = m.norm
    blocked = ops.is_b8(x)
    if not blocked and x.shape[-1] != m.conv.in_channels:
        assert x.dtype == torch.float32 and in_ab is None
        pc = packed_conv_padded_in(cache, m.conv, x.shape[-1])
    else:
        pc = packed_conv(cache, m.conv, x.dtype)
    if blocked:
        N, _, H, W, _ = x.shape
    else:
        N, H, W, _ = x.shape
    wino = x.dtype == torch.float32 and ops.wino_eligible(pc, H, W, x.dtype) and pc.Cin <= 512
    if blocked and not wino:
        x = ops.gn_apply_b8(x, *(in_ab if in_ab is not None else (None, None)), relu=in_relu and in_ab is not None)
        in_ab, blocked = None, False
    OH, OW = pc.out_hw(H, W)
    fused_stats = wino or (OH * OW) % 128 == 0
    fuse_in = in_ab is not None and (wino or ((H * W) % 128 == 0 and pc.stride == 1 and (OH, OW) == (H, W)
                                              and x.dtype == torch.float32))
    if fuse_in and not wino and save is None and pc.KH * pc.KW > 1:
        fuse_in = False
    if in_ab is not None and not fuse_in:
        x = ops.gn_apply(x, in_ab[0], in_ab[1], relu=in_relu, out=x if (consume_input and save is None) else None)
        in_ab = None
    out_b8 = bool(out_b8) and wino and save is None and not materialize
    bias = m.conv.bias
    if fused_stats:
        raw, part = ops.conv2d(x, pc, bias=bias, in_ab=in_ab, in_relu=in_relu, gn_part=True, out_b8=out_b8)
    else:
        raw = ops.conv2d(x, pc, bias=bias, in_ab=in_ab, in_relu=in_relu)
        part = ops.gn_stats(raw)
    if save is not None:
        a, b, mean, rstd = ops.gn_finalize(part, gn.weight, gn.bias, N, OH * OW, gn.num_groups, gn.eps, want_stats=True)
        save.update(module=m, x=x, in_ab=in_ab, in_relu=in_relu, raw=raw, a=a, b=b, mean=mean, rstd=rstd)
    else:
        a, b = ops.gn_finalize(part, gn.weight, gn.bias, N, OH * OW, gn.num_groups, gn.eps)
    if not materialize:
        return raw, (a, b)
    return ops.gn_apply(raw, a, b, relu=m.with_activation, up=up, out=None if save is not None else raw)
```

### pointtinybenchmark_amd/necks/fpn.py

```python
import warnings

import torch.nn as nn

from .. import ops
from ..layers import ConvModule, _PackCache, conv_gn
from ..registry import NECKS


@NECKS.register_module()
class FPN(nn.Module):
    def __init__(self, in_channels, out_channels, num_outs, start_level=0, end_level=-1, add_extra_convs=False,
                 extra_convs_on_inputs=True, relu_before_extra_convs=False, no_norm_on_lateral=False, conv_cfg=None,
                 norm_cfg=None, act_cfg=None, upsample_cfg=dict(mode='nearest'), init_cfg=None):
        super().__init__()
        assert isinstance(in_channels, (list, tuple))
        assert norm_cfg is not None and norm_cfg['type'] == 'GN' and not no_norm_on_lateral and act_cfg is None, \
            'the CPR/P2P configs use GN laterals without activation (SURVEY.md §8 a2)'
        assert upsample_cfg.get('mode', 'nearest') == 'nearest' and 'scale_factor' not in upsample_cfg
        self.in_channels, self.out_channels, self.num_outs = list(in_channels), out_channels, num_outs
        self.num_ins = len(in_channels)
        self.backbone_end_level = self.num_ins if end_level == -1 else end_level
        self.start_level, self.end_level = start_level, end_level
        self.relu_before_extra_convs = relu_before_extra_convs
        if end_level != -1:
            assert end_level <= len(in_channels)
            assert num_outs <= end_level - start_level, 'extra pyramid levels need end_level == -1'
        assert isinstance(add_extra_convs, (str, bool))
        if isinstance(add_extra_convs, str):
            assert add_extra_convs in ('on_input', 'on_lateral', 'on_output')
        elif add_extra_convs:
            if extra_convs_on_inputs:
                warnings.warn("add_extra_convs=True with extra_convs_on_inputs is deprecated: pass add_extra_convs='on_input'",
                              DeprecationWarning)
                add_extra_convs = 'on_input'
            else:
                add_extra_convs = 'on_output'
        self.add_extra_convs = add_extra_convs
        self.lateral_convs = nn.ModuleList()
        self.fpn_convs = nn.ModuleList()
        for i in range(start_level, self.backbone_end_level):
            self.lateral_convs.append(ConvModule(in_channels[i], out_channels, 1, norm_cfg=norm_cfg, act_cfg=None))
            if i < start_level + num_outs:
                self.fpn_convs.append(ConvModule(out_channels, out_channels, 3, padding=1, norm_cfg=norm_cfg,
                                                 act_cfg=None))
        self.extra_levels = max(0, num_outs - self.backbone_end_level + start_level)
        if self.add_extra_convs:
            for k in range(self.extra_levels):
                cin = in_channels[self.backbone_end_level - 1] if k == 0 and self.add_extra_convs == 'on_input' else out_channels
                self.fpn_convs.append(ConvModule(cin, out_channels, 3, stride=2, padding=1, norm_cfg=norm_cfg, act_cfg=None))
        self._cache = _PackCache()
        self.init_weights()

    def init_weights(self):
        for m in self.modules():
            if isinstance(m, nn.Conv2d):
                nn.init.xavier_uniform_(m.weight)
                if m.bias is not None:
                    nn.init.constant_(m.bias, 0)

    def run_laterals(self, xs, tape=None):
        c = self._cache
        lat = [None] * len(xs)
        for i in range(len(xs) - 1, -1, -1):
            up = lat[i + 1] if i + 1 < len(xs) else None
            rec = None
            if tape is not None:
                rec = dict(kind='lateral', level=i)
                tape.append(rec)
            lat[i] = conv_gn(c, self.lateral_convs[i], xs[i], up=up, save=rec)
        return lat

    def run_outputs(self, lat, src, lazy, tape=None, out_b8=False):
        c, outs = self._cache, []
        for i in range(min(len(lat), self.num_outs)):
            rec = None
            if tape is not None:
                rec = dict(kind='out', level=i)
                tape.append(rec)
            outs.append(conv_gn(c, self.fpn_convs[i], lat[i], materialize=not lazy, save=rec,
                                out_b8=out_b8 and lazy and not self.extra_levels))
        if self.extra_levels:
            assert len(lat) == len(self.lateral_convs) and (src is not None) == (self.add_extra_convs == 'on_input')
            outs += self.run_extras(outs[-1], lat[-1], src, lazy, tape)
        return outs

    def _run(self, inputs, lazy, tape=None, out_b8=False):
        assert len(inputs) == len(self.in_channels)
        xs = [ops.neck_input(inputs[i + self.start_level]) for i in range(len(self.lateral_convs))]
        lat = self.run_laterals(xs, tape)
        src = None
        if self.extra_levels and self.add_extra_convs == 'on_input':
            src = ops.neck_input(inputs[self.backbone_end_level - 1])
        return self.run_outputs(lat, src, lazy, tape, out_b8)

    def run_extras(self, last, lat_last, src, lazy, tape=None):
        c, outs, used = self._cache, [], len(self.lateral_convs)
        if not self.add_extra_convs:
            for k in range(self.extra_levels):
                if tape is not None:
                    tape.append(dict(kind='pool', level=used + k))
                if lazy:
                    last = (ops.subsample2(last[0]), last[1])
                else:
                    last = ops.subsample2(last)
                outs.append(last)
            return outs
        cur = None
        for k in range(self.extra_levels):
            relu = k > 0 and self.relu_before_extra_convs
            reads = self.add_extra_convs if k == 0 else 'on_output'
            if reads == 'on_input':
                x = src
            elif reads == 'on_lateral':
                x = lat_last
            elif k == 0 and not lazy:
                x = last
            else:
                raw, (a, b) = last if k == 0 else cur
                x = ops.gn_apply(raw, a, b, relu=relu)
            rec = None
            if tape is not None:
                rec = dict(kind='extra', level=used + k, reads=reads, relu_in=relu)
                tape.append(rec)
            cur = conv_gn(c, self.fpn_convs[used + k], x, materialize=False, save=rec)
            outs.append(cur if lazy else ops.gn_apply(cur[0], cur[1][0], cur[1][1]))
        return outs

    def forward(self, inputs):
        return tuple(ops.as_nchw(t) for t in self._run(inputs, lazy=False))

    def forward_lazy(self, inputs, tape=None, out_b8=False):
        return self._run(inputs, lazy=True, tape=tape, out_b8=out_b8 and tape is None)
```

### pointtinybenchmark_amd/ops.py

```python
import collections
import ctypes
import math

import torch

from . import _lib


def _ptr(t):
    return ctypes.c_void_p(t.data_ptr()) if t is not None else None


def _stream():
    return ctypes.c_void_p(torch.cuda.current_stream().cuda_stream)


def _check(t, dtype=torch.float32):
    if not t.is_cuda:
        raise _lib.CprHipError('HIP op called with a CPU tensor: the product path has no CPU fallback')
    ok = t.dtype in dtype if isinstance(dtype, tuple) else t.dtype == dtype
    assert ok and t.is_contiguous(), (t.dtype, t.stride())
    return t


# ... 3 lines not shown
def as_nchw(x_nhwc):
    return x_nhwc.permute(0, 3, 1, 2)


def pad32(c):
    return (c + 31) // 32 * 32


def as_nchw_padded(buf, C):
    if buf.shape[-1] == C:
        return as_nchw(buf)
    view = buf[..., :C].permute(0, 3, 1, 2)
    view._cpr_padded = buf
    return view


def padded_buffer(x):
    buf = getattr(x, '_cpr_padded', None)
    if buf is None:
        return None
    N, C, H, W = x.shape
    ok = buf.dim() == 4 and tuple(buf.shape[:3]) == (N, H, W) and buf.shape[3] == pad32(C) and buf.is_contiguous() and \
        x.data_ptr() == buf.data_ptr() and x.stride() == (H * W * buf.shape[3], 1, W * buf.shape[3], buf.shape[3])
    return buf if ok else None


def from_nchw(x):
    y = x.permute(0, 2, 3, 1)
    if y.is_contiguous():
        return y
    return nchw_to_nhwc(x)


NECK_INPUT_COPIES = [0]


def neck_input(x):
    C = x.shape[1]
    if C % 32 == 0 or C <= 4:
        return from_nchw(x)
    buf = padded_buffer(x)
    if buf is None:
        N, _, H, W = x.shape
        buf = torch.zeros((N, H, W, pad32(C)), device=x.device, dtype=torch.float32)
        buf[..., :C].copy_(x.permute(0, 2, 3, 1))
        NECK_INPUT_COPIES[0] += 1
    return buf


def nchw_to_nhwc(x):
    N, C, H, W = x.shape
    if C <= 4:
        x = _check(x.contiguous())
        out = torch.empty((N, H, W, 4), device=x.device, dtype=torch.float32)
        _lib.call('cpr_nchw_to_nhwc4', _ptr(x), _ptr(out), N, C, H, W, _stream())
        return out
    return x.permute(0, 2, 3, 1).contiguous()


def nhwc_to_nchw_dense(x_nhwc):
    N, H, W, C = x_nhwc.shape
    out = torch.empty((N, C, H, W), device=x_nhwc.device, dtype=torch.float32)
    _lib.call('cpr_nhwc_to_nchw', _ptr(_check(x_nhwc)), _ptr(out), N, C, H, W, _stream())
    return out


class PackedConv:
    wfrag = None
    wino = None
    wino32 = None
    ready = None
    groups = 1
    cg = None
    C = None
    dilation = 1

    def _packed(self):
        self.ready = record_ready()

    def __init__(self, weight, stride=1, padding=0, dtype=torch.float32, groups=1, pitch=None, dilation=1):
        dilation = int(dilation)
        assert dilation >= 1, 'dilation must be >= 1, got %d' % dilation
        if dilation != 1 and dtype == torch.bfloat16:
            raise NotImplementedError('dilation=%d: a dilated convolution runs in the fp32 compute mode only (the bf16 kernels have no '
                                      'dilated form)' % dilation)
        if groups > 1:
            self._init_grouped(weight, stride, padding, dtype, groups, None, 0, pitch, dilation)
            return
        assert pitch is None, 'a channel pitch is the grouped kernels\' (dense layers pad their packs)'
        Cout, Cin, KH, KW = weight.shape
        if dilation != 1:
            assert (KH, KW) == (3, 3) and stride == 1 and padding == dilation and Cin % 32 == 0, \
                'dilation=%d: 3x3 / stride 1 / padding == dilation with Cin %% 32 == 0, got weight %s stride %d padding %d' \
                % (dilation, tuple(weight.shape), stride, padding)
            self.dilation = dilation
        w = weight.detach().to(torch.float32).permute(0, 2, 3, 1)
        self.dtype = dtype
        if dtype == torch.bfloat16:
            assert Cin % 64 == 0, 'bf16 conv needs Cin % 64 == 0'
            self.Cout, self.Cin, self.KH, self.KW, self.Kpad = Cout, Cin, KH, KW, KH * KW * Cin
            self.stride, self.padding = stride, padding
            if weight.is_cuda:
                self._pack_bf16(weight, None, 0)
                return
            self.w = w.reshape(Cout, KH * KW * Cin).to(torch.bfloat16).contiguous()
            return
        if Cin <= 4:
            cin_p = 4
        else:
            assert Cin % 32 == 0, 'input channels must be a multiple of 32 (or <= 4 for the stem)'
            cin_p = Cin
        K = KH * KW * cin_p
        Kpad = (K + 31) // 32 * 32
        self.Cout, self.Cin, self.KH, self.KW, self.Kpad = Cout, cin_p, KH, KW, Kpad
        self.stride, self.padding = stride, padding
        if weight.is_cuda:
            src = weight.detach()
            if src.dtype != torch.float32 or not src.is_contiguous():
                src = src.float().contiguous()
            self.w = torch.empty((Cout, Kpad), device=weight.device, dtype=torch.float32)
            _lib.call('cpr_pack_weights', _ptr(src), None, _ptr(self.w), Cout, Cin, KH, KW, cin_p, Kpad, 0, _stream())
            self._packed()
            return
        wp = torch.zeros((Cout, KH, KW, cin_p), device=weight.device, dtype=torch.float32)
        wp[..., :Cin] = w
        packed = torch.zeros((Cout, Kpad), device=weight.device, dtype=torch.float32)
        packed[:, :K] = wp.reshape(Cout, K)
        self.w = packed.contiguous()

    def _init_grouped(self, weight, stride, padding, dtype, groups, scale, transpose, pitch=None, dilation=1):
        C, cg, KH, KW = weight.shape
        pitch = C if pitch is None else int(pitch)
        assert pitch >= C and pitch % 4 == 0, 'grouped conv: the channel pitch %d must be a multiple of 4 and >= C = %d' % (pitch, C)
        if dtype != torch.float32:
            raise NotImplementedError('a grouped convolution (groups=%d) runs in the fp32 compute mode only, not in %s' % (groups, dtype))
        assert weight.is_cuda, 'the grouped pack is built on the device'
        assert cg * groups == C and cg in GROUP_WIDTHS and (KH, KW) == (3, 3) and padding == dilation and stride in (1, 2), \
            'grouped conv: 3x3 / padding == dilation / stride 1 or 2 with a group width in %s, got weight %s groups %d stride %d ' \
            'padding %d dilation %d' % (GROUP_WIDTHS, tuple(weight.shape), groups, stride, padding, dilation)
        assert dilation == 1 or (stride == 1 and pitch == C), \
            'grouped conv: dilation=%d needs stride 1 and unpitched maps, got stride %d pitch %d (C = %d)' % (dilation, stride, pitch, C)
        self.dtype, self.groups, self.cg, self.C = torch.float32, groups, cg, C
        self.Cout, self.Cin, self.KH, self.KW, self.Kpad = pitch, pitch, 3, 3, 9 * cg
        self.stride, self.padding = stride, dilation
        if dilation != 1:
            self.dilation = dilation
        src = weight.detach()
        if src.dtype != torch.float32 or not src.is_contiguous():
            src = src.float().contiguous()
        self.w = torch.empty((9 * cg * C,), device=weight.device, dtype=torch.float32)
        _lib.call('cpr_pack_weights_grouped', _ptr(src), _ptr(scale), _ptr(self.w), C, cg, int(transpose), _stream())
        self._packed()

    @staticmethod
    def dgrad_padding(k, padding, dilation=1):
        return dilation * (k - 1) - padding

    @classmethod
    def for_dgrad_grouped(cls, weight, groups, scale=None, pitch=None, dilation=1):
        self = cls.__new__(cls)
        self._init_grouped(weight, 1, self.dgrad_padding(3, dilation, dilation), torch.float32, groups, scale, 1, pitch, dilation)
        return self

    def _pack_bf16(self, weight, scale, transpose):
        src = weight.detach()
        if src.dtype != torch.float32 or not src.is_contiguous():
            src = src.float().contiguous()
        O, I, KH, KW = src.shape
        rows = self.Cout
        self.w = torch.empty((rows, self.Kpad), device=src.device, dtype=torch.bfloat16)
        want_frag = rows % 256 == 0 and self.Kpad % 64 == 0 and WFRAG[0]
        if want_frag:
            self.wfrag = torch.empty((rows // 64, self.Kpad // 16, 2, 2, 32, 8), device=src.device, dtype=torch.bfloat16)
        _lib.call('cpr_pack_weights_bf16', _ptr(src), _ptr(scale), _ptr(self.w), _ptr(self.wfrag if want_frag else None), O, I, KH, KW,
                  int(transpose), _stream())
        self._packed()

    @classmethod
    def for_dgrad_bf16(cls, weight, padding, scale=None, pad_override=None):
        Cout, Cin, KH, KW = weight.shape
        assert (KH == KW or pad_override is not None) and weight.is_cuda and Cout % 64 == 0
        self = cls.__new__(cls)
        self.dtype = torch.bfloat16
        self.Cout, self.Cin, self.KH, self.KW, self.Kpad = Cin, Cout, KH, KW, KH * KW * Cout
        self.stride, self.padding = 1, (KH - 1 - padding if pad_override is None else pad_override)
        self._pack_bf16(weight, scale, 1)
        return self

    def frag_image(self):
        if self.dtype != torch.bfloat16 or self.Cout % 256 != 0 or self.Kpad % 64 != 0 or not WFRAG[0]:
            return None
        if self.wfrag is None:
            G, KS = self.Cout // 64, self.Kpad // 16
            self.wfrag = self.w.view(G, 32, 2, KS, 2, 8).permute(0, 3, 2, 4, 1, 5).contiguous()
            self._packed()
        return self.wfrag

    @classmethod
    def for_dgrad(cls, weight, padding, scale=None, pad_override=None, dilation=1):
        Cout, Cin, KH, KW = weight.shape
        assert (KH == KW or pad_override is not None) and weight.is_cuda
        dilation = int(dilation)
        assert dilation == 1 or ((KH, KW) == (3, 3) and pad_override is None and padding == dilation and Cout % 32 == 0), \
            'dilation=%d: the data gradient of a 3x3 / padding == dilation layer, got weight %s padding %d' \
            % (dilation, tuple(weight.shape), padding)
        assert Cout % 32 == 0 or Cout <= 4, 'gradient channels must be a multiple of 32 (or <= 4)'
        self = cls.__new__(cls)
        self.dtype = torch.float32
        cols_p = 4 if Cout <= 4 else Cout
        K = KH * KW * cols_p
        Kpad = (K + 31) // 32 * 32
        self.Cout, self.Cin, self.KH, self.KW, self.Kpad = Cin, cols_p, KH, KW, Kpad
        self.stride, self.padding = 1, (self.dgrad_padding(KH, padding, dilation) if pad_override is None else pad_override)
        if dilation != 1:
            self.dilation = dilation
        src = weight.detach()
        if src.dtype != torch.float32 or not src.is_contiguous():
            src = src.float().contiguous()
        self.w = torch.empty((Cin, Kpad), device=weight.device, dtype=torch.float32)
        _lib.call('cpr_pack_weights', _ptr(src), _ptr(scale), _ptr(self.w), Cout, Cin, KH, KW, cols_p, Kpad, 1, _stream())
        self._packed()
        return self

    def out_hw(self, H, W):
        d = self.dilation
        return ((H + 2 * self.padding - d * (self.KH - 1) - 1) // self.stride + 1,
                (W + 2 * self.padding - d * (self.KW - 1) - 1) // self.stride + 1)


CONV_RELU, CONV_OUT_BF16, CONV_RES_MASK, CONV_COLSUM = 1, 2, 4, 8
GROUP_WIDTHS = (4, 8, 16, 24, 32, 40, 48, 56)
WFRAG = [True]
TRACE_CONV_VARIANT = [False, None]

WINOGRAD = [True]
WINO_MIN_FILL = 0.6


def record_ready():
    if not torch.cuda.is_available() or torch.cuda.is_current_stream_capturing():
        return None
    ev = torch.cuda.Event()
    ev.record()
    return ev, torch.cuda.current_stream().cuda_stream


def wait_ready(ready):
    if ready is None or torch.cuda.is_current_stream_capturing():
        return ready
    ev, stream = ready
    if ev.query():
        return None
    cur = torch.cuda.current_stream()
    if cur.cuda_stream != stream:
        cur.wait_event(ev)
    return ready


def pack_ready(pc):
    if pc.ready is not None:
        pc.ready = wait_ready(pc.ready)


def wino_eligible(pc, H, W, dtype=torch.float32):
    if pc.dilation != 1:
        return False
    if not (pc.groups == 1 and WINOGRAD[0] and dtype == torch.float32 and pc.dtype == torch.float32 and pc.KH == 3 and pc.KW == 3 and
            pc.stride == 1 and pc.padding == 1 and pc.Cin % 16 == 0 and pc.Cin >= 32 and pc.Cout % 64 == 0):
        return False
    fill = (H * W) / float(((H + 15) // 16 * 16) * ((W + 15) // 16 * 16))
    return fill >= WINO_MIN_FILL


WINO_TILE = ['auto']


def wino_instance(pc, H, W, fused_affine):
    can32 = pc.Cin % 8 == 0 and (not fused_affine or pc.Cin <= 256)
    if WINO_TILE[0] == '64' or not can32:
        return '64'
    if WINO_TILE[0] == '32':
        return '32'
    return WINO_AUTO(pc, H, W, fused_affine)


WINO32_MAX_PIXELS = 40 * 40


def WINO_AUTO(pc, H, W, fused_affine):
    return '32' if H * W <= WINO32_MAX_PIXELS else '64'


def wino_gn_slots(pc, H, W, fused_affine):
    if wino_instance(pc, H, W, fused_affine) == '32':
        return ((H + 7) // 8) * ((W + 15) // 16)
    return ((H + 15) // 16) * ((W + 15) // 16)


def is_b8(x):
    return x.dim() == 5 and x.shape[-1] == 8


def conv3x3_wino(x, pc, scale=None, bias=None, relu=False, gn_part=False, out=None, in_ab=None, in_relu=False,
                 out_b8=False):
    _check(x, ACT)
    in_b8 = is_b8(x)
    if in_b8:
        N, _, H, W, _ = x.shape
        Cin = x.shape[1] * 8
    else:
        N, H, W, Cin = x.shape
    assert x.dtype == torch.float32 and Cin == pc.Cin and pc.KH == 3 and pc.stride == 1 and pc.padding == 1
    inst = wino_instance(pc, H, W, in_ab is not None)
    attr, pack_fn = ('wino32', 'cpr_wino32_pack_weights') if inst == '32' else ('wino', 'cpr_wino_pack_weights')
    if getattr(pc, attr) is None:
        pack_ready(pc)
        wino = torch.empty((16 * pc.Cin * pc.Cout,), device=x.device, dtype=torch.float32)
        _lib.call(pack_fn, _ptr(pc.w), _ptr(wino), pc.Cin, pc.Cout, pc.Kpad, _stream())
        setattr(pc, attr, wino)
        pc._packed()
    pack_ready(pc)
    shape = (N, pc.Cout // 8, H, W, 8) if out_b8 else (N, H, W, pc.Cout)
    if out is None:
        out = torch.empty(shape, device=x.device, dtype=torch.float32)
    assert tuple(out.shape) == shape and out.is_contiguous()
    part = None
    if gn_part:
        part = torch.empty((N * wino_gn_slots(pc, H, W, in_ab is not None), pc.Cout, 2), device=x.device, dtype=torch.float32)
    a = b = None
    if in_ab is not None:
        a, b = in_ab
        assert Cin <= 512
    _lib.call('cpr_conv3x3_wino32_fwd' if inst == '32' else 'cpr_conv3x3_wino_fwd', _ptr(x), _ptr(getattr(pc, attr)), _ptr(out),
              _ptr(scale), _ptr(bias), _ptr(a), _ptr(b), _ptr(part), N, H, W, Cin, pc.Cout, CONV_RELU if relu else 0, int(in_relu),
              (1 if in_b8 else 0) | (2 if out_b8 else 0), _stream())
    if TRACE_CONV_VARIANT[0]:
        TRACE_CONV_VARIANT[1] = ('wino32' if inst == '32' else 'wino',
                                 (1 if in_b8 else 0) | (2 if out_b8 else 0) | (4 if in_ab is not None else 0))
    return (out, part) if gn_part else out


def gn_apply_b8(x, a=None, b=None, relu=False):
    assert is_b8(x)
    N, C8, H, W, _ = _check(x, ACT).shape
    y = torch.empty((N, H, W, C8 * 8), device=x.device, dtype=torch.float32)
    _lib.call('cpr_gn_apply_b8', _ptr(x), _ptr(a), _ptr(b), _ptr(y), N, H, W, C8 * 8, int(relu), _stream())
    return y


def conv2d(x, pc, scale=None, bias=None, residual=None, relu=False, in_ab=None, in_relu=False, gn_part=False,
           out=None, out_dtype=None, res_mask=False, colsum=False, out_b8=False):
    _check(x, ACT)
    pack_ready(pc)
    if is_b8(x):
        assert residual is None and not (res_mask or colsum) and out_dtype in (None, torch.float32) and \
            wino_eligible(pc, x.shape[2], x.shape[3], x.dtype), 'channel-blocked input needs a Winograd-eligible layer'
        return conv3x3_wino(x, pc, scale, bias, relu, gn_part, out, in_ab, in_relu, out_b8)
    N, H, W, Cin = x.shape
    assert Cin == pc.Cin, (Cin, pc.Cin)
    assert x.dtype == pc.dtype, 'weights were packed for %s, input is %s' % (pc.dtype, x.dtype)
    OH, OW = pc.out_hw(H, W)
    odt = out_dtype or x.dtype
    if pc.groups > 1:
        assert residual is None and in_ab is None and not (in_relu or gn_part or res_mask or colsum or out_b8) and \
            odt == torch.float32, 'the grouped conv has no residual, GroupNorm-statistics, fused-input-affine or bf16 form'
        if out is None:
            out = torch.empty((N, OH, OW, pc.Cout), device=x.device, dtype=torch.float32)
        assert tuple(out.shape) == (N, OH, OW, pc.Cout) and out.is_contiguous()
        if scale is not None or bias is not None:
            assert (scale is None or _check(scale).numel() >= pc.C) and (bias is None or _check(bias).numel() >= pc.C)
        if pc.dilation != 1:
            assert Cin == pc.C and pc.stride == 1
            _lib.call('cpr_conv_group_fwd_dil', _ptr(x), _ptr(pc.w), _ptr(out), _ptr(scale), _ptr(bias), N, H, W, Cin, pc.cg, pc.dilation,
                      CONV_RELU if relu else 0, _stream())
        elif Cin == pc.C:
            _lib.call('cpr_conv_group_fwd', _ptr(x), _ptr(pc.w), _ptr(out), _ptr(scale), _ptr(bias), N, H, W, Cin, pc.cg, pc.stride,
                      CONV_RELU if relu else 0, _stream())
        else:
            _lib.call('cpr_conv_group_fwd_pitch', _ptr(x), _ptr(pc.w), _ptr(out), _ptr(scale), _ptr(bias), N, H, W, pc.C, Cin, pc.cg,
                      pc.stride, CONV_RELU if relu else 0, _stream())
        if TRACE_CONV_VARIANT[0]:
            TRACE_CONV_VARIANT[1] = ('group', pc.cg)
        return out
    if residual is None and not (res_mask or colsum) and odt == torch.float32 and wino_eligible(pc, H, W, x.dtype) and \
            (in_ab is None or Cin <= 512):
        return conv3x3_wino(x, pc, scale, bias, relu, gn_part, out, in_ab, in_relu, out_b8)
    assert not out_b8, 'channel-blocked output is produced by the Winograd layers only (check wino_eligible first)'
    if pc.dilation != 1:
        assert in_ab is None and not (in_relu or gn_part) and odt == torch.float32 and x.dtype == torch.float32, \
            'a dilated conv (dilation=%d) has no fused-input-affine, GroupNorm-statistics or bf16 form' % pc.dilation
        if out is None:
            out = torch.empty((N, OH, OW, pc.Cout), device=x.device, dtype=torch.float32)
        assert tuple(out.shape) == (N, OH, OW, pc.Cout) and out.is_contiguous()
        part = torch.empty(((N * OH * OW + 63) // 64, pc.Cout, 2), device=x.device, dtype=torch.float32) if colsum else None
        variant = ctypes.c_int(0) if (colsum or TRACE_CONV_VARIANT[0]) else None
        flags = (CONV_RELU if relu else 0) | (CONV_RES_MASK if res_mask else 0) | (CONV_COLSUM if colsum else 0)
        _lib.call('cpr_conv2d_fwd_dil', _ptr(x), _ptr(pc.w), _ptr(out), _ptr(scale), _ptr(bias), _ptr(residual), None, None, _ptr(part),
                  N, H, W, Cin, pc.Cout, pc.KH, pc.KW, pc.stride, pc.padding, pc.dilation, pc.Kpad, flags, 0,
                  ctypes.byref(variant) if variant is not None else None, _stream())
        if variant is not None:
            TRACE_CONV_VARIANT[1] = ('fp32_dil', variant.value)
        if colsum:
            bm = variant.value // 1000000
            return out, TilePartials(part, (N * OH * OW + bm - 1) // bm, pc.Cout)
        return out
    if out is None:
        out = torch.empty((N, OH, OW, pc.Cout), device=x.device, dtype=odt)
    part = None
    if gn_part:
        assert (OH * OW) % 128 == 0 and not colsum
        part = torch.empty((N * OH * OW // 128, pc.Cout, 2), device=x.device, dtype=torch.float32)
    if colsum and x.dtype != torch.bfloat16:
        part = torch.empty(((N * OH * OW + 63) // 64, pc.Cout, 2), device=x.device, dtype=torch.float32)
    variant = ctypes.c_int(0) if (colsum or TRACE_CONV_VARIANT[0]) else None
    vref = ctypes.byref(variant) if variant is not None else None
    if x.dtype == torch.bfloat16:
        assert in_ab is None, 'the bf16 kernel does not fuse the producer GroupNorm (materialise with gn_apply)'
        if res_mask or colsum:
            assert res_mask and colsum and residual is not None and residual.dtype == torch.bfloat16 and not relu and not gn_part
            slots = conv2d_bf16_mask_slots(x.shape, pc, odt)
            assert slots > 0, 'this shape has no mask-mode instance (ask conv2d_bf16_mask_slots first)'
            part = torch.empty((slots, pc.Cout, 2), device=x.device, dtype=torch.float32)
            _lib.call('cpr_conv2d_fwd_bf16', _ptr(x), _ptr(pc.w), _ptr(pc.frag_image()), _ptr(out), _ptr(scale), _ptr(bias), _ptr(residual),
                      _ptr(part), N, H, W, Cin, pc.Cout, pc.KH, pc.KW, pc.stride, pc.padding, pc.Kpad, 2,
                      int(odt == torch.float32), vref, _stream())
            if variant is not None:
                TRACE_CONV_VARIANT[1] = ('bf16', variant.value)
            return out, TilePartials(part, slots, pc.Cout)
        _lib.call('cpr_conv2d_fwd_bf16', _ptr(x), _ptr(pc.w), _ptr(pc.frag_image()), _ptr(out), _ptr(scale), _ptr(bias), _ptr(residual),
                  _ptr(part), N, H, W, Cin, pc.Cout, pc.KH, pc.KW, pc.stride, pc.padding, pc.Kpad, int(relu),
                  int(odt == torch.float32), vref, _stream())
        if variant is not None:
            TRACE_CONV_VARIANT[1] = ('bf16', variant.value)
        return (out, part) if gn_part else out
    a = b = None
    if in_ab is not None:
        a, b = in_ab
    flags = (CONV_RELU if relu else 0) | (CONV_OUT_BF16 if odt == torch.bfloat16 else 0) | \
        (CONV_RES_MASK if res_mask else 0) | (CONV_COLSUM if colsum else 0)
    _lib.call('cpr_conv2d_fwd', _ptr(x), _ptr(pc.w), _ptr(out), _ptr(scale), _ptr(bias),
              _ptr(residual), _ptr(a), _ptr(b), _ptr(part), N, H, W, Cin, pc.Cout, pc.KH, pc.KW, pc.stride,
              pc.padding, pc.Kpad, flags, int(in_relu), vref, _stream())
    if variant is not None:
        TRACE_CONV_VARIANT[1] = ('fp32', variant.value)
    if colsum:
        bm = variant.value // 1000000
        return out, TilePartials(part, (N * OH * OW + bm - 1) // bm, pc.Cout)
    return (out, part) if gn_part else out


def conv2d_bf16_mask_slots(x_shape, pc, out_dtype=torch.bfloat16, fused_add=False):
    N, H, W, Cin = x_shape
    if pc.groups > 1 or (fused_add and (not WFRAG[0] or pc.Cout % 256 != 0)):
        return 0
    return _lib.call('cpr_conv2d_bf16_mask_slots', N, H, W, Cin, pc.Cout, pc.KH, pc.KW, pc.stride, pc.padding,
                     2 if fused_add else int(out_dtype == torch.float32), positive=True)


def conv2d_dgrad_bf16_fused(g16, pc, mask, add):
    _check(g16, ACT)
    pack_ready(pc)
    N, H, W, Cin = g16.shape
    OH, OW = pc.out_hw(H, W)
    shape = (N, OH, OW, pc.Cout)
    assert g16.dtype == torch.bfloat16 and pc.dtype == torch.bfloat16 and Cin == pc.Cin
    assert mask.dtype == torch.bfloat16 and add.dtype == torch.float32 and tuple(mask.shape) == shape and tuple(add.shape) == shape
    assert mask.is_contiguous() and add.is_contiguous()
    slots = conv2d_bf16_mask_slots(g16.shape, pc, fused_add=True)
    assert slots > 0, 'this shape has no fused instance (ask conv2d_bf16_mask_slots(..., fused_add=True) first)'
    out32 = torch.empty(shape, device=g16.device, dtype=torch.float32)
    out16 = torch.empty(shape, device=g16.device, dtype=torch.bfloat16)
    part = torch.empty((slots, pc.Cout, 2), device=g16.device, dtype=torch.float32)
    variant = ctypes.c_int(0) if TRACE_CONV_VARIANT[0] else None
    _lib.call('cpr_conv2d_dgrad_bf16_fused', _ptr(g16), _ptr(pc.w), _ptr(pc.frag_image()), _ptr(out32), _ptr(out16), _ptr(add), _ptr(mask),
              _ptr(part), N, H, W, Cin, pc.Cout, pc.KH, pc.KW, pc.stride, pc.padding, pc.Kpad,
              ctypes.byref(variant) if variant is not None else None, _stream())
    if variant is not None:
        TRACE_CONV_VARIANT[1] = ('bf16', variant.value)
    return out32, out16, TilePartials(part, slots, pc.Cout)


def conv1x1_stream(x, pc, scale=None, bias=None, residual=None, relu=False, res_mask=False):
    N, H, W, Cin = x.shape
    assert pc.KH == 1 and pc.stride == 1 and pc.padding == 0 and pc.Kpad == Cin and x.dtype == torch.float32
    out = torch.empty((N, H, W, pc.Cout), device=x.device, dtype=torch.float32)
    flags = (CONV_RELU if relu else 0) | (CONV_RES_MASK if res_mask else 0)
    _lib.call('cpr_conv1x1_stream_fwd', _ptr(x), _ptr(pc.w), _ptr(out), _ptr(scale), _ptr(bias), _ptr(residual),
              N * H * W, Cin, pc.Cout, flags, _stream())
    return out


def conv2d_dual(x, pc, x2, pc2, scale=None, bias=None, scale2=None, bias2=None, relu=False, out=None):
    _check(x, ACT)
    _check(x2, ACT)
    pack_ready(pc)
    pack_ready(pc2)
    N, H, W, Cin = x.shape
    N2, H2, W2, Cin2 = x2.shape
    assert x.dtype == torch.float32 and x2.dtype == torch.float32 and pc.dtype == torch.float32 and pc2.dtype == torch.float32
    assert N == N2 and Cin == pc.Cin and Cin2 == pc2.Cin and pc.Cout == pc2.Cout and pc2.KH == 1 and pc2.KW == 1 and pc2.padding == 0
    OH, OW = pc.out_hw(H, W)
    assert (OH, OW) == pc2.out_hw(H2, W2), 'the two sources must produce the same output grid'
    if out is None:
        out = torch.empty((N, OH, OW, pc.Cout), device=x.device, dtype=torch.float32)
    variant = ctypes.c_int(0) if TRACE_CONV_VARIANT[0] else None
    _lib.call('cpr_conv2d_dual_fwd', _ptr(x), _ptr(pc.w), _ptr(x2), _ptr(pc2.w), _ptr(out), _ptr(scale), _ptr(bias),
              _ptr(scale2), _ptr(bias2), N, H, W, Cin, pc.Cout, pc.KH, pc.KW, pc.stride, pc.padding, pc.Kpad, H2, W2, Cin2,
              pc2.stride, pc2.Kpad, CONV_RELU if relu else 0, ctypes.byref(variant) if variant is not None else None, _stream())
    if variant is not None:
        TRACE_CONV_VARIANT[1] = ('fp32', variant.value)
    return out


class TilePartials:

    def __init__(self, part, tiles, C):
        self.part, self.tiles, self.C = part, tiles, C

    def record_stream(self, stream):
        self.part.record_stream(stream)

    def reduce(self):
        cs = torch.empty((self.C,), device=self.part.device, dtype=torch.float32)
        ws = torch.empty((64 * self.C,), device=self.part.device, dtype=torch.float32)
        _lib.call('cpr_part_colsum', _ptr(self.part), _ptr(cs), _ptr(ws), self.tiles, self.C, _stream())
        return cs


def _sfx(x):
    return '_bf16' if x.dtype == torch.bfloat16 else ''


def bn_fold(gamma, beta, mean, var, eps, want_inv_sigma=False):
    C = gamma.numel()
    dev = gamma.device
    scale = torch.empty((C,), device=dev, dtype=torch.float32)
    shift = torch.empty((C,), device=dev, dtype=torch.float32)
    inv = torch.empty((C,), device=dev, dtype=torch.float32) if want_inv_sigma else None
    _lib.call('cpr_bn_fold', _ptr(_check(gamma.detach())), _ptr(_check(beta.detach())), _ptr(_check(mean)), _ptr(_check(var)),
              float(eps), _ptr(scale), _ptr(shift), _ptr(inv), C, _stream())
    return scale, shift, inv


def _bn_rows(y):
    C = y.shape[-1]
    M = y.numel() // C
    if M <= 1:
        raise ValueError('Expected more than 1 value per channel when training, got input size %s' % (tuple(y.shape),))
    assert C % 64 == 0, 'training-mode BatchNorm needs C % 64 == 0, got %d' % C
    return M, C


def _bn_vec(t, C):
    if t is None:
        return None
    t = _check(t.detach())
    assert t.numel() == C, 'per-channel vector of %d elements, want %d' % (t.numel(), C)
    return t


BnStats = collections.namedtuple('BnStats', 'mean rstd scale shift center cmean cshift')


def bn_batch_stats(y, gamma, beta, running_mean=None, running_var=None, num_batches_tracked=None, momentum=0.1, eps=1e-5, group=None):
    if sync_world_size(group) > 1:
        rec, _ = bn_sync_local_stats(y)
        return bn_sync_merge_stats(_sync_gather(rec, group), y, gamma, beta, running_mean, running_var, num_batches_tracked, momentum, eps)
    M, C = _bn_rows(_check(y))
    dev = y.device
    st = torch.empty((7, C), device=dev, dtype=torch.float32)
    ws = torch.empty((_lib.call('cpr_bn_train_ws', M, C, positive=True),), device=dev, dtype=torch.float32)
    if momentum is None:
        assert num_batches_tracked is not None, 'momentum None averages over num_batches_tracked'
    assert (running_mean is None) == (running_var is None), 'running_mean and running_var go together'
    bufs = [t for t in (running_mean, running_var) if t is not None]
    for t in bufs:
        _bn_vec(t, C)
    if num_batches_tracked is not None:
        assert _check(num_batches_tracked, torch.int64).numel() == 1
    _lib.call('cpr_bn_batch_stats', _ptr(y), _ptr(_bn_vec(gamma, C)), _ptr(_bn_vec(beta, C)), _ptr(running_mean),
              _ptr(running_var), _ptr(num_batches_tracked), -1.0 if momentum is None else float(momentum), float(eps),
              _ptr(st[0]), _ptr(st[1]), _ptr(st[2]), _ptr(st[3]), _ptr(st[4]), _ptr(st[5]), _ptr(st[6]), _ptr(ws), M, C, _stream())
    from torch.autograd.graph import increment_version
    for t in bufs + ([num_batches_tracked] if num_batches_tracked is not None else []):
        increment_version(t)
    return BnStats(*st.unbind(0))


def bn_apply(y, scale, shift, residual=None, relu=False, center=None, y2=None, scale2=None, shift2=None, center2=None, out=None):
    M, C = y.numel() // _check(y).shape[-1], y.shape[-1]
    for t in (residual, y2):
        if t is not None:
            assert _check(t).shape == y.shape, (t.shape, y.shape)
    assert residual is None or y2 is None
    assert y2 is not None or (scale2 is None and shift2 is None and center2 is None), 'scale2 / shift2 / center2 belong to y2'
    assert y2 is None or (scale2 is not None and shift2 is not None), 'the two-input form needs scale2 and shift2'
    if out is None:
        out = torch.empty_like(y)
    assert _check(out).shape == y.shape
    _lib.call('cpr_bn_apply', _ptr(y), _ptr(_bn_vec(center, C)), _ptr(_bn_vec(scale, C)), _ptr(_bn_vec(shift, C)), _ptr(residual),
              _ptr(y2), _ptr(_bn_vec(center2, C)), _ptr(_bn_vec(scale2, C)), _ptr(_bn_vec(shift2, C)), _ptr(out), M, C, int(relu),
              _stream())
    return out


def bn_train_bwd(dout, y, mean, rstd, gamma, mask=None, out_dgamma=None, out_dbeta=None, center=None, group=None, count=None):
    if sync_world_size(group) > 1:
        assert count is not None, 'the synchronised backward divides by the global row count of the forward (BnSyncStats.count)'
        rec, ws, dg, db = bn_sync_local_bwd(dout, y, mean, rstd, mask=mask, out_dgamma=out_dgamma, out_dbeta=out_dbeta, center=center)
        return bn_sync_merge_bwd(_sync_gather(rec, group), ws, count, dout, y, mean, rstd, gamma, mask=mask, center=center), dg, db
    M, C = _bn_rows(_check(y))
    assert _check(dout).shape == y.shape and (mask is None or _check(mask).shape == y.shape)
    dev = y.device
    dg = out_dgamma if out_dgamma is not None else torch.empty((C,), device=dev, dtype=torch.float32)
    db = out_dbeta if out_dbeta is not None else torch.empty((C,), device=dev, dtype=torch.float32)
    dy = torch.empty_like(y)
    ws = torch.empty((_lib.call('cpr_bn_train_ws', M, C, positive=True),), device=dev, dtype=torch.float32)
    _lib.call('cpr_bn_train_bwd', _ptr(dout), _ptr(mask), _ptr(y), _ptr(_bn_vec(center, C)), _ptr(_bn_vec(mean, C)), _ptr(_bn_vec(rstd, C)),
              _ptr(_bn_vec(gamma, C)), _ptr(dy), _ptr(_bn_vec(dg, C)), _ptr(_bn_vec(db, C)), _ptr(ws), M, C, _stream())
    return dy, dg, db


class BnSyncStats(BnStats):
    count = None


def sync_world_size(group=None):
    if group is None:
        return 1
    import torch.distributed as dist
    if not (dist.is_available() and dist.is_initialized()):
        return 1
    return dist.get_world_size(group)


def _sync_gather(record, group):
    import torch.distributed as dist
    R = dist.get_world_size(group)
    out = torch.empty((R * record.numel(),), device=record.device, dtype=record.dtype)
    dist.all_gather_into_tensor(out, record, group=group)
    return out.view(R, record.numel())


def _bn_sync_rows(y):
    C = y.shape[-1]
    M = y.numel() // C if C else 0
    if M < 1:
        raise ValueError('SyncBN: this rank holds no rows (input size %s): every rank of the group brings at least one value per channel'
                         % (tuple(y.shape),))
    assert C % 64 == 0, 'training-mode BatchNorm needs C % 64 == 0, got %d' % C
    return M, C


def _bn_sync_records(records, n, y):
    assert _check(records, torch.float64).dim() == 2 and records.shape[1] == n, (tuple(records.shape), n)
    assert records.device == y.device
    return int(records.shape[0])


def bn_sync_local_stats(y):
    M, C = _bn_sync_rows(_check(y))
    rec = torch.empty((2 * C + 1,), device=y.device, dtype=torch.float64)
    ws = torch.empty((_lib.call('cpr_bn_sync_ws', M, C, positive=True),), device=y.device, dtype=torch.float32)
    _lib.call('cpr_bn_sync_stats_local', _ptr(y), _ptr(rec), _ptr(ws), M, C, _stream())
    return rec, ws


def bn_sync_merge_stats(records, y, gamma, beta, running_mean=None, running_var=None, num_batches_tracked=None, momentum=0.1, eps=1e-5):
    M, C = _bn_sync_rows(_check(y))
    R = _bn_sync_records(records, 2 * C + 1, y)
    if R == 1 and M <= 1:
        raise ValueError('Expected more than 1 value per channel when training, got input size %s' % (tuple(y.shape),))
    dev = y.device
    st = torch.empty((7, C), device=dev, dtype=torch.float32)
    count = torch.empty((1,), device=dev, dtype=torch.float64)
    if momentum is None:
        assert num_batches_tracked is not None, 'momentum None averages over num_batches_tracked'
    assert (running_mean is None) == (running_var is None), 'running_mean and running_var go together'
    bufs = [t for t in (running_mean, running_var) if t is not None]
    for t in bufs:
        _bn_vec(t, C)
    if num_batches_tracked is not None:
        assert _check(num_batches_tracked, torch.int64).numel() == 1
    _lib.call('cpr_bn_sync_stats_merge', _ptr(records), R, _ptr(y), _ptr(_bn_vec(gamma, C)), _ptr(_bn_vec(beta, C)), _ptr(running_mean),
              _ptr(running_var), _ptr(num_batches_tracked), -1.0 if momentum is None else float(momentum), float(eps),
              _ptr(st[0]), _ptr(st[1]), _ptr(st[2]), _ptr(st[3]), _ptr(st[4]), _ptr(st[5]), _ptr(st[6]), _ptr(count), C, _stream())
    from torch.autograd.graph import increment_version
    for t in bufs + ([num_batches_tracked] if num_batches_tracked is not None else []):
        increment_version(t)
# ... 1321 lines not shown
```

Baseline: 912.3.

## Fuse FPN level-0 lateral GN affine and nearest upsample-add into Winograd conv load

```diff
diff --git a/include/cpr_hip.h b/include/cpr_hip.h
--- a/include/cpr_hip.h
+++ b/include/cpr_hip.h
@@ -40,6 +40,9 @@
 int cpr_conv3x3_wino_fwd(const float* in, const float* u, float* out, const float* scale, const float* bias,
                          const float* in_a, const float* in_b, float* gn_part, int N, int H, int W, int Cin, int Cout,
                          int flags, int in_relu, int layout, void* stream);
+int cpr_conv3x3_wino_fwd_up(const float* in, const float* u, float* out, const float* scale, const float* bias,
+                            const float* in_a, const float* in_b, float* gn_part, int N, int H, int W, int Cin, int Cout,
+                            int flags, int in_relu, int layout, const float* up, int UH, int UW, void* stream);
 int cpr_wino32_pack_weights(const float* wgt, float* u, int Cin, int Cout, int Kpad, void* stream);
 int cpr_conv3x3_wino32_slots(int H, int W);
 int cpr_conv3x3_wino32_fwd(const float* in, const float* u, float* out, const float* scale, const float* bias,
diff --git a/pointtinybenchmark_amd/_lib.py b/pointtinybenchmark_amd/_lib.py
--- a/pointtinybenchmark_amd/_lib.py
+++ b/pointtinybenchmark_amd/_lib.py
@@ -20,6 +20,7 @@
     'cpr_conv_wgrad_bf16_s': [_p, _i, _p, _i, _p, _p] + [_i] * 8 + [_p],
     'cpr_wino_pack_weights': [_p, _p, _i, _i, _i, _p],
     'cpr_conv3x3_wino_fwd': [_p, _p, _p, _p, _p, _p, _p, _p, _i, _i, _i, _i, _i, _i, _i, _i, _p],
+    'cpr_conv3x3_wino_fwd_up': [_p, _p, _p, _p, _p, _p, _p, _p, _i, _i, _i, _i, _i, _i, _i, _i, _p, _i, _i, _p],
     'cpr_wino32_pack_weights': [_p, _p, _i, _i, _i, _p],
     'cpr_conv3x3_wino32_slots': [_i, _i],
     'cpr_conv3x3_wino32_fwd': [_p, _p, _p, _p, _p, _p, _p, _p, _i, _i, _i, _i, _i, _i, _i, _i, _p],
diff --git a/pointtinybenchmark_amd/csrc/conv_wino.hip b/pointtinybenchmark_amd/csrc/conv_wino.hip
--- a/pointtinybenchmark_amd/csrc/conv_wino.hip
+++ b/pointtinybenchmark_amd/csrc/conv_wino.hip
@@ -30,6 +30,8 @@
     float* gn_part;
     const float* in_a;
     const float* in_b;
+    const float* up;
+    int UH, UW;
     int in_relu, out_b8;
     int N, H, W, Cin, Cout, relu, RY, RX, regions, tilesN, nch;
     int tpx;
@@ -65,8 +67,9 @@
     }
 }
 
-template <int ABL, bool INB8, bool XF, int TSPREAD = 1, int VAR = 0>
-__global__ __launch_bounds__(512, 1) void conv_wino_kernel(WinoParams p) {
+template <int ABL, bool INB8, bool XF, int TSPREAD, int VAR, bool UP>
+__device__ __forceinline__ void conv_wino_body(const WinoParams& p) {
+    static_assert(!UP || (XF && !INB8), "the upsampled addend comes with the affine on an NHWC input");
     constexpr bool DEEP = (VAR & 1) != 0, UDMA = (VAR & 4) != 0, USINGLE = (VAR & 2) != 0 && !UDMA;
     constexpr int XFMAX = 512;
     constexpr int RAWROW = 148;
@@ -86,6 +89,9 @@
         const_cast<float*>(p.in), 0, (int)((size_t)p.N * p.H * p.W * p.Cin * 4), 0x00020000);
     const __amdgpu_buffer_rsrc_t rs_u = __builtin_amdgcn_make_buffer_rsrc(
         const_cast<float*>(p.u), 0, (int)((size_t)p.tilesN * p.nch * WBUF * 4), 0x00020000);
+    const __amdgpu_buffer_rsrc_t rs_up = __builtin_amdgcn_make_buffer_rsrc(
+        const_cast<float*>(UP ? p.up : nullptr), 0, UP ? (int)((size_t)p.N * p.UH * p.UW * p.Cin * 4) : 0, 0x00020000);
+    const float up_sy = UP ? (float)p.UH / (float)p.H : 0.f, up_sx = UP ? (float)p.UW / (float)p.W : 0.f;
     float* Rw = smem + 4 * WBUF;
     float* ABs = smem + 4 * WBUF + 2 * RAWBUF;
     int par = 0;
@@ -108,6 +114,7 @@
     struct Tile {
         int rg, tn, n, oy0, ox0, n0;
         int voffA[2];
+        int voffU[2];
         unsigned uok;
         bool any_pad, valid;
     };
@@ -142,12 +149,17 @@
             const bool ok = (k == 0 || unit1_live) & ((unsigned)iy < (unsigned)p.H) & ((unsigned)ix < (unsigned)p.W);
             t.uok |= (ok ? 1u : 0u) << k;
             t.voffA[k] = ok ? img_base + (iy * p.W + ix) * pixbytes + (tid & 1) * 16 : (int)0x80000000;
+            if (UP) {
+                const int uy = min((int)floorf(iy * up_sy), p.UH - 1), ux = min((int)floorf(ix * up_sx), p.UW - 1);
+                t.voffU[k] = ok ? ((t.n * p.UH + uy) * p.UW + ux) * pixbytes + (tid & 1) * 16 : (int)0x80000000;
+            }
         }
         t.any_pad = XF && __builtin_amdgcn_ballot_w64(t.uok != (unit1_live ? 3u : 1u)) != 0;
         return t;
     };
 
     f32x4 sp[2][2];
+    f32x4 spu[UP ? 2 : 1][2];
     f32x4 su[(USINGLE || UDMA) ? 1 : 2][4];
     float tab_a = 0.f, tab_b = 0.f;
     f32x2 d[4][2];
@@ -156,6 +168,9 @@
     auto ld_a = [&](const Tile& t, int ck, int k) {
         return __builtin_bit_cast(f32x4, __builtin_amdgcn_raw_buffer_load_b128(rs_in, t.voffA[k], ck * chunk_bytes, 0));
     };
+    auto ld_up = [&](const Tile& t, int ck, int k) {
+        return __builtin_bit_cast(f32x4, __builtin_amdgcn_raw_buffer_load_b128(rs_up, t.voffU[k], ck * 32, 0));
+    };
     auto ld_u = [&](const Tile& t, int ck, int z) {
         return __builtin_bit_cast(
             f32x4, __builtin_amdgcn_raw_buffer_load_b128(rs_u, tid * 16 + z * 8192, (t.tn * p.nch + ck) * (WBUF * 4), 0));
@@ -164,6 +179,10 @@
         if (!(ABL & 8)) {
             sp[0][0] = ld_a(t, 0, 0); sp[1][0] = ld_a(t, 1, 0);
             if (second_unit) { sp[0][1] = ld_a(t, 0, 1); sp[1][1] = ld_a(t, 1, 1); }
+            if (UP) {
+                spu[0][0] = ld_up(t, 0, 0); spu[UP ? 1 : 0][0] = ld_up(t, 1, 0);
+                if (second_unit) { spu[0][1] = ld_up(t, 0, 1); spu[UP ? 1 : 0][1] = ld_up(t, 1, 1); }
+            }
         }
         if (!UDMA) {
 #pragma unroll
@@ -178,6 +197,12 @@
         if (ABL & 8) return;
         const int ck = chunk < last ? chunk : last;
         if (k == 0 || second_unit) sp[SET][k] = ld_a(cur, ck, k);
+    };
+    auto g_up = [&](auto set_c, int chunk, int k) {
+        constexpr int SET = UP ? decltype(set_c)::value : 0;
+        if (!UP || (ABL & 8)) return;
+        const int ck = chunk < last ? chunk : last;
+        if (k == 0 || second_unit) spu[SET][k] = ld_up(cur, ck, k);
     };
     auto g_u = [&](auto set_c, int chunk, int z) {
         constexpr int SET = (USINGLE || UDMA) ? 0 : decltype(set_c)::value;
@@ -194,19 +219,24 @@
                      :: "s"(m0v), "v"(tid * 16 + z * 8192), "s"(rs_u_raw), "s"(soff) : "memory");
     };
     auto dma_wait = [&](auto npatch_c) {
-        constexpr int NP = decltype(npatch_c)::value;
+        constexpr int NP = decltype(npatch_c)::value * (UP ? 2 : 1);
         if (NP == 0) asm volatile("s_waitcnt vmcnt(0)" ::: "memory");
         else if (second_unit) asm volatile("s_waitcnt vmcnt(%0)" :: "n"(2 * NP) : "memory");
         else asm volatile("s_waitcnt vmcnt(%0)" :: "n"(NP) : "memory");
     };
-    auto affine = [&](f32x4 v, f32x4 a4, f32x4 b4, int k) {
+    auto affine = [&](f32x4 v, f32x4 a4, f32x4 b4, int k, f32x4 u4) {
         if (ABL & 64) v = v * a4 + b4;
         else {
             const f32x2 lo = pk_fma(f32x2{v.x, v.y}, f32x2{a4.x, a4.y}, f32x2{b4.x, b4.y});
             const f32x2 hi = pk_fma(f32x2{v.z, v.w}, f32x2{a4.z, a4.w}, f32x2{b4.z, b4.w});
             v = f32x4{lo.x, lo.y, hi.x, hi.y};
         }
-        v.x = fmaxf(v.x, relu_floor); v.y = fmaxf(v.y, relu_floor); v.z = fmaxf(v.z, relu_floor); v.w = fmaxf(v.w, relu_floor);
+        if (UP) {
+            const f32x2 lo = pk_add(f32x2{v.x, v.y}, f32x2{u4.x, u4.y}), hi = pk_add(f32x2{v.z, v.w}, f32x2{u4.z, u4.w});
+            v = f32x4{lo.x, lo.y, hi.x, hi.y};
+        } else {
+            v.x = fmaxf(v.x, relu_floor); v.y = fmaxf(v.y, relu_floor); v.z = fmaxf(v.z, relu_floor); v.w = fmaxf(v.w, relu_floor);
+        }
         if (cur.any_pad) {
             asm volatile("");
             if (!((cur.uok >> k) & 1u)) v = f32x4{0.f, 0.f, 0.f, 0.f};
@@ -223,7 +253,7 @@
         constexpr int SET = decltype(set_c)::value;
         if (k == 1 && !second_unit) return;
         f32x4 v = sp[SET][k];
-        if (XF) v = affine(v, xa4, xb4, k);
+        if (XF) v = affine(v, xa4, xb4, k, UP ? spu[UP ? SET : 0][k] : f32x4{});
         if (k == 0 || unit1_live) *reinterpret_cast<f32x4*>(Rw + buf * RAWBUF + raw_wr[k]) = v;
     };
     auto r_a_pro = [&](int chunk01, int k) {
@@ -231,7 +261,8 @@
         f32x4 v = chunk01 ? sp[1][k] : sp[0][k];
         if (XF) {
             const float* tab = ABs + par * 2 * XFMAX + chunk01 * 8 + (tid & 1) * 4;
-            v = affine(v, *reinterpret_cast<const f32x4*>(tab), *reinterpret_cast<const f32x4*>(tab + XFMAX), k);
+            v = affine(v, *reinterpret_cast<const f32x4*>(tab), *reinterpret_cast<const f32x4*>(tab + XFMAX), k,
+                       !UP ? f32x4{} : chunk01 ? spu[UP ? 1 : 0][k] : spu[0][k]);
         }
         if (k == 0 || unit1_live) *reinterpret_cast<f32x4*>(Rw + chunk01 * RAWBUF + raw_wr[k]) = v;
     };
@@ -311,7 +342,8 @@
 #pragma unroll
     for (int z = 0; z < 4; ++z) r_u(Set0{}, 0, z);
     g_a(Set0{}, 2, 0); g_a(Set0{}, 2, 1);
-    if (DEEP) { g_a(Set1{}, 3, 0); g_a(Set1{}, 3, 1); }
+    g_up(Set0{}, 2, 0); g_up(Set0{}, 2, 1);
+    if (DEEP) { g_a(Set1{}, 3, 0); g_a(Set1{}, 3, 1); g_up(Set1{}, 3, 0); g_up(Set1{}, 3, 1); }
 #pragma unroll
     for (int z = 0; z < 4; ++z) g_u(Set0{}, USINGLE ? 1 : 2, z);
     __syncthreads();
@@ -385,10 +417,14 @@
                 if (UDMA) {
                     if (q < 4 && c + 2 < p.nch) dma_u(c + 2, buf, q);
                     if (q == 4) g_a(pset_c, c + (DEEP ? 4 : 3), 0);
+                    if (q == 5) g_up(pset_c, c + (DEEP ? 4 : 3), 0);
                     if (q == 6) g_a(pset_c, c + (DEEP ? 4 : 3), 1);
+                    if (q == 7) g_up(pset_c, c + (DEEP ? 4 : 3), 1);
                 } else {
                     if (q == 3) g_a(pset_c, c + (DEEP ? 4 : 3), 0);
+                    if (q == 4) g_up(pset_c, c + (DEEP ? 4 : 3), 0);
                     if (q == 5) g_a(pset_c, c + (DEEP ? 4 : 3), 1);
+                    if (q == 6) g_up(pset_c, c + (DEEP ? 4 : 3), 1);
                     if (q == 7) g_u(nxt_c, c + (USINGLE ? 2 : 3), 3);
                 }
                 if (TSPREAD == 1 && q >= 4) t_read(buf, q - 4);
@@ -492,6 +528,15 @@
     }
 }
 
+template <int ABL, bool INB8, bool XF, int TSPREAD = 1, int VAR = 0>
+__global__ __launch_bounds__(512, 1) void conv_wino_kernel(WinoParams p) {
+    conv_wino_body<ABL, INB8, XF, TSPREAD, VAR, false>(p);
+}
+template <int TSPREAD, int VAR>
+__global__ __launch_bounds__(512, 1) void conv_wino_up_kernel(WinoParams p) {
+    conv_wino_body<0, false, true, TSPREAD, VAR, true>(p);
+}
+
 #ifdef CPR_BENCH_HOOKS
 static int wino_sched = 0, wino_ablate = 0, wino_var = -1, wino_tpx = -1;
 extern "C" int cpr_wino_set_variant(int sched, int ablate) {
@@ -516,16 +561,20 @@
     CPR_LAUNCH_STATUS();
 }
 static int wino_fwd_launch(const float* in, const float* u, float* out, const float* scale, const float* bias,
-                           const float* in_a, const float* in_b, float* gn_part, int N, int H, int W, int Cin,
-                           int Cout, int flags, int in_relu, int layout, hipStream_t stream) {
+                           const float* in_a, const float* in_b, const float* up, int UH, int UW, float* gn_part, int N,
+                           int H, int W, int Cin, int Cout, int flags, int in_relu, int layout, hipStream_t stream) {
     CPR_CHECK_ARG(in && u && out && N > 0 && H > 0 && W > 0);
     CPR_CHECK_ARG(Cin > 0 && Cout > 0 && Cin % 16 == 0 && Cout % 64 == 0 && Cin >= 32);
     CPR_CHECK_ARG((flags & ~CPR_CONV_RELU) == 0 && (layout & ~3) == 0);
     if (in_a) CPR_CHECK_ARG(in_b && Cin <= 512);
+    if (up) {
+        CPR_CHECK_ARG(in_a && in_b && !in_relu && !(layout & CPR_WINO_IN_B8) && UH > 0 && UW > 0);
+        if ((long long)N * UH * UW * Cin * 4 >= (1ll << 31)) return CPR_ERR_UNSUPPORTED;
+    }
     if ((long long)N * H * W * Cin * 4 >= (1ll << 31) || (long long)N * H * W * Cout * 4 >= (1ll << 31)) return CPR_ERR_UNSUPPORTED;
     WinoParams p;
     p.in = in; p.u = u; p.out = out; p.scale = scale; p.bias = bias; p.gn_part = gn_part;
-    p.in_a = in_a; p.in_b = in_b; p.in_relu = in_relu; p.out_b8 = (layout & CPR_WINO_OUT_B8) ? 1 : 0;
+    p.in_a = in_a; p.in_b = in_b; p.up = up; p.UH = UH; p.UW = UW; p.in_relu = in_relu; p.out_b8 = (layout & CPR_WINO_OUT_B8) ? 1 : 0;
     p.N = N; p.H = H; p.W = W; p.Cin = Cin; p.Cout = Cout; p.relu = flags & CPR_CONV_RELU;
     p.RY = (H + 15) / 16; p.RX = (W + 15) / 16;
     p.regions = N * p.RY * p.RX; p.tilesN = Cout / 64; p.nch = Cin / 8;
@@ -561,6 +610,9 @@
         else hipLaunchKernelGGL((conv_wino_kernel<A_, false, false, TP_, V_>), dim3(grid), dim3(512), 0, stream, p);              \
     } while (0)
 #define WLAUNCH(A_, F_) WLAUNCHV(A_, F_, WINO_VAR_DEFAULT)
+    if (up) {
+        hipLaunchKernelGGL((conv_wino_up_kernel<0, WINO_VAR_DEFAULT>), dim3(grid), dim3(512), 0, stream, p);
+    } else
 #ifdef CPR_BENCH_HOOKS
     if ((var != WINO_VAR_DEFAULT || wino_sched == 2) && !wino_ablate) {
         switch (var * 3 + wino_sched) {
@@ -598,9 +650,9 @@
     CPR_LAUNCH_STATUS();
 }
 
-extern "C" int cpr_conv3x3_wino_fwd(const float* in, const float* u, float* out, const float* scale, const float* bias,
-                                    const float* in_a, const float* in_b, float* gn_part, int N, int H, int W, int Cin,
-                                    int Cout, int flags, int in_relu, int layout, hipStream_t stream) {
+static int wino_fwd_split(const float* in, const float* u, float* out, const float* scale, const float* bias, const float* in_a,
+                          const float* in_b, const float* up, int UH, int UW, float* gn_part, int N, int H, int W, int Cin,
+                          int Cout, int flags, int in_relu, int layout, hipStream_t stream) {
     CPR_CHECK_ARG(N > 0 && H > 0 && W > 0 && Cin > 0 && Cout > 0);
     const int per = cpr_images_per_launch(N, (long long)H * W * cpr_max2(Cin, Cout) * 4);
     if (per <= 0) return CPR_ERR_UNSUPPORTED;
@@ -609,9 +661,24 @@
         const int n = N - n0 < per ? N - n0 : per;
         const int rc = wino_fwd_launch(in + (size_t)n0 * H * W * Cin, u, out + (size_t)n0 * H * W * Cout, scale, bias,
                                        in_a ? in_a + (size_t)n0 * Cin : nullptr, in_b ? in_b + (size_t)n0 * Cin : nullptr,
+                                       up ? up + (size_t)n0 * UH * UW * Cin : nullptr, UH, UW,
                                        gn_part ? gn_part + (size_t)n0 * slots * Cout * 2 : nullptr, n, H, W, Cin, Cout, flags,
                                        in_relu, layout, stream);
         if (rc != CPR_OK) return rc;
     }
     return CPR_OK;
 }
+extern "C" int cpr_conv3x3_wino_fwd(const float* in, const float* u, float* out, const float* scale, const float* bias,
+                                    const float* in_a, const float* in_b, float* gn_part, int N, int H, int W, int Cin,
+                                    int Cout, int flags, int in_relu, int layout, hipStream_t stream) {
+    return wino_fwd_split(in, u, out, scale, bias, in_a, in_b, nullptr, 0, 0, gn_part, N, H, W, Cin, Cout, flags, in_relu, layout,
+                          stream);
+}
+extern "C" int cpr_conv3x3_wino_fwd_up(const float* in, const float* u, float* out, const float* scale, const float* bias,
+                                       const float* in_a, const float* in_b, float* gn_part, int N, int H, int W, int Cin,
+                                       int Cout, int flags, int in_relu, int layout, const float* up, int UH, int UW,
+                                       hipStream_t stream) {
+    CPR_CHECK_ARG(up && in_a && in_b && !in_relu && !(layout & CPR_WINO_IN_B8) && UH > 0 && UW > 0);
+    return wino_fwd_split(in, u, out, scale, bias, in_a, in_b, up, UH, UW, gn_part, N, H, W, Cin, Cout, flags, in_relu, layout,
+                          stream);
+}
diff --git a/pointtinybenchmark_amd/layers.py b/pointtinybenchmark_amd/layers.py
--- a/pointtinybenchmark_amd/layers.py
+++ b/pointtinybenchmark_amd/layers.py
@@ -260,7 +260,7 @@
 
 
 def conv_gn(cache, m, x, in_ab=None, in_relu=False, materialize=True, up=None, save=None, consume_input=False,
-            out_b8=False):
+            out_b8=False, in_up=None):
     gn = m.norm
     blocked = ops.is_b8(x)
     if not blocked and x.shape[-1] != m.conv.in_channels:
@@ -282,13 +282,14 @@
                                               and x.dtype == torch.float32))
     if fuse_in and not wino and save is None and pc.KH * pc.KW > 1:
         fuse_in = False
+    assert in_up is None or (wino and fuse_in and not in_relu and save is None and not blocked), 'in_up needs a fused Winograd load'
     if in_ab is not None and not fuse_in:
         x = ops.gn_apply(x, in_ab[0], in_ab[1], relu=in_relu, out=x if (consume_input and save is None) else None)
         in_ab = None
     out_b8 = bool(out_b8) and wino and save is None and not materialize
     bias = m.conv.bias
     if fused_stats:
-        raw, part = ops.conv2d(x, pc, bias=bias, in_ab=in_ab, in_relu=in_relu, gn_part=True, out_b8=out_b8)
+        raw, part = ops.conv2d(x, pc, bias=bias, in_ab=in_ab, in_relu=in_relu, gn_part=True, out_b8=out_b8, in_up=in_up)
     else:
         raw = ops.conv2d(x, pc, bias=bias, in_ab=in_ab, in_relu=in_relu)
         part = ops.gn_stats(raw)
diff --git a/pointtinybenchmark_amd/necks/fpn.py b/pointtinybenchmark_amd/necks/fpn.py
--- a/pointtinybenchmark_amd/necks/fpn.py
+++ b/pointtinybenchmark_amd/necks/fpn.py
@@ -1,10 +1,16 @@
+import collections
 import warnings
 
+import torch
 import torch.nn as nn
 
 from .. import ops
-from ..layers import ConvModule, _PackCache, conv_gn
+from ..layers import ConvModule, _PackCache, conv_gn, packed_conv
 from ..registry import NECKS
+
+FUSE_LEVEL0 = [True]
+
+LazyLateral = collections.namedtuple('LazyLateral', 'raw ab up')
 
 
 @NECKS.register_module()
@@ -58,7 +64,17 @@
                 if m.bias is not None:
                     nn.init.constant_(m.bias, 0)
 
-    def run_laterals(self, xs, tape=None):
+    def lazy_level0(self, xs, tape=None):
+        if not FUSE_LEVEL0[0] or tape is not None or len(xs) < 2 or type(self).run_outputs is not FPN.run_outputs:
+            return False
+        x = xs[0]
+        if x.dtype != torch.float32 or not self.fpn_convs:
+            return False
+        pc = packed_conv(self._cache, self.fpn_convs[0].conv, torch.float32)
+        H, W = x.shape[1], x.shape[2]
+        return ops.wino_eligible(pc, H, W, torch.float32) and pc.Cin <= 512 and ops.wino_instance(pc, H, W, True) == '64'
+
+    def run_laterals(self, xs, tape=None, lazy0=False):
         c = self._cache
         lat = [None] * len(xs)
         for i in range(len(xs) - 1, -1, -1):
@@ -67,7 +83,11 @@
             if tape is not None:
                 rec = dict(kind='lateral', level=i)
                 tape.append(rec)
-            lat[i] = conv_gn(c, self.lateral_convs[i], xs[i], up=up, save=rec)
+            if i == 0 and lazy0:
+                assert tape is None and up is not None
+                lat[0] = LazyLateral(*conv_gn(c, self.lateral_convs[0], xs[0], materialize=False), up)
+            else:
+                lat[i] = conv_gn(c, self.lateral_convs[i], xs[i], up=up, save=rec)
         return lat
 
     def run_outputs(self, lat, src, lazy, tape=None, out_b8=False):
@@ -77,8 +97,11 @@
             if tape is not None:
                 rec = dict(kind='out', level=i)
                 tape.append(rec)
-            outs.append(conv_gn(c, self.fpn_convs[i], lat[i], materialize=not lazy, save=rec,
-                                out_b8=out_b8 and lazy and not self.extra_levels))
+            x, pending = lat[i], {}
+            if isinstance(x, LazyLateral):
+                x, pending = x.raw, dict(in_ab=x.ab, in_up=x.up)
+            outs.append(conv_gn(c, self.fpn_convs[i], x, materialize=not lazy, save=rec,
+                                out_b8=out_b8 and lazy and not self.extra_levels, **pending))
         if self.extra_levels:
             assert len(lat) == len(self.lateral_convs) and (src is not None) == (self.add_extra_convs == 'on_input')
             outs += self.run_extras(outs[-1], lat[-1], src, lazy, tape)
@@ -87,7 +110,7 @@
     def _run(self, inputs, lazy, tape=None, out_b8=False):
         assert len(inputs) == len(self.in_channels)
         xs = [ops.neck_input(inputs[i + self.start_level]) for i in range(len(self.lateral_convs))]
-        lat = self.run_laterals(xs, tape)
+        lat = self.run_laterals(xs, tape, lazy0=self.lazy_level0(xs, tape))
         src = None
         if self.extra_levels and self.add_extra_convs == 'on_input':
             src = ops.neck_input(inputs[self.backbone_end_level - 1])
diff --git a/pointtinybenchmark_amd/ops.py b/pointtinybenchmark_amd/ops.py
--- a/pointtinybenchmark_amd/ops.py
+++ b/pointtinybenchmark_amd/ops.py
@@ -329,7 +329,7 @@
 
 
 def conv3x3_wino(x, pc, scale=None, bias=None, relu=False, gn_part=False, out=None, in_ab=None, in_relu=False,
-                 out_b8=False):
+                 out_b8=False, in_up=None):
     _check(x, ACT)
     in_b8 = is_b8(x)
     if in_b8:
@@ -358,6 +358,15 @@
     if in_ab is not None:
         a, b = in_ab
         assert Cin <= 512
+    if in_up is not None:
+        assert not in_b8 and in_ab is not None and not in_relu and inst == '64', (in_b8, in_ab is None, in_relu, inst)
+        assert _check(in_up, ACT).dtype == torch.float32 and in_up.dim() == 4 and in_up.shape[0] == N and in_up.shape[3] == Cin
+        _lib.call('cpr_conv3x3_wino_fwd_up', _ptr(x), _ptr(pc.wino), _ptr(out), _ptr(scale), _ptr(bias), _ptr(a), _ptr(b), _ptr(part),
+                  N, H, W, Cin, pc.Cout, CONV_RELU if relu else 0, 0, 2 if out_b8 else 0, _ptr(in_up), in_up.shape[1],
+                  in_up.shape[2], _stream())
+        if TRACE_CONV_VARIANT[0]:
+            TRACE_CONV_VARIANT[1] = ('wino', (2 if out_b8 else 0) | 4 | 8)
+        return (out, part) if gn_part else out
     _lib.call('cpr_conv3x3_wino32_fwd' if inst == '32' else 'cpr_conv3x3_wino_fwd', _ptr(x), _ptr(getattr(pc, attr)), _ptr(out),
               _ptr(scale), _ptr(bias), _ptr(a), _ptr(b), _ptr(part), N, H, W, Cin, pc.Cout, CONV_RELU if relu else 0, int(in_relu),
               (1 if in_b8 else 0) | (2 if out_b8 else 0), _stream())
@@ -376,12 +385,13 @@
 
 
 def conv2d(x, pc, scale=None, bias=None, residual=None, relu=False, in_ab=None, in_relu=False, gn_part=False,
-           out=None, out_dtype=None, res_mask=False, colsum=False, out_b8=False):
+           out=None, out_dtype=None, res_mask=False, colsum=False, out_b8=False, in_up=None):
     _check(x, ACT)
     pack_ready(pc)
     if is_b8(x):
         assert residual is None and not (res_mask or colsum) and out_dtype in (None, torch.float32) and \
             wino_eligible(pc, x.shape[2], x.shape[3], x.dtype), 'channel-blocked input needs a Winograd-eligible layer'
+        assert in_up is None, 'the upsampled addend needs an NHWC input'
         return conv3x3_wino(x, pc, scale, bias, relu, gn_part, out, in_ab, in_relu, out_b8)
     N, H, W, Cin = x.shape
     assert Cin == pc.Cin, (Cin, pc.Cin)
@@ -411,7 +421,8 @@
         return out
     if residual is None and not (res_mask or colsum) and odt == torch.float32 and wino_eligible(pc, H, W, x.dtype) and \
             (in_ab is None or Cin <= 512):
-        return conv3x3_wino(x, pc, scale, bias, relu, gn_part, out, in_ab, in_relu, out_b8)
+        return conv3x3_wino(x, pc, scale, bias, relu, gn_part, out, in_ab, in_relu, out_b8, in_up)
+    assert in_up is None, 'only the Winograd layers add an upsampled map on load (check wino_eligible / wino_instance first)'
     assert not out_b8, 'channel-blocked output is produced by the Winograd layers only (check wino_eligible first)'
     if pc.dilation != 1:
         assert in_ab is None and not (in_relu or gn_part) and odt == torch.float32 and x.dtype == torch.float32, \
```

Measured after the change: 909.4. About the same (-0.3%).
